# alexlee-gk/video_prediction

Hardware: AMD Instinct MI355X
Metric: train frames/sec (whole node), BAIR 64x64 seq30 SAVP (higher is better)
Workload: dtype bf16

## Files before the change

### include/savp_hip.h

```cpp
#ifndef SAVP_HIP_H
#define SAVP_HIP_H

#include <stdint.h>

#ifdef __cplusplus
extern "C" {
#endif

#define SAVP_OK 0
#define SAVP_EINVAL (-1)
#define SAVP_ELAUNCH (-2)

const char* savp_version(void);

int savp_set_option(const char* name, int32_t value);
int savp_get_option(const char* name, int32_t* value);

int savp_allreduce_bucket(void* comm, void* stream, void* buf, int64_t count);

int savp_prof_event_create(void** ev);
int savp_prof_event_destroy(void* ev);
int savp_prof_arm(void* start, void* stop);
int savp_prof_armed(void);
int savp_prof_elapsed_us(void* start, void* stop, float* us);

enum { SAVP_CONV_FPROP = 0, SAVP_CONV_DGRAD = 1, SAVP_CONV_WGRAD = 2 };
enum { SAVP_PREC_F32 = 0, SAVP_PREC_BF16 = 1 };
enum { SAVP_ACT_NONE = 0, SAVP_ACT_LRELU = 1, SAVP_ACT_SIGMOID = 2, SAVP_ACT_DLRELU_FROM_OUT = 3 };

typedef struct SavpConvArgs {
    int32_t mode;
    int32_t N, D, H, W, Cx;
    int32_t Do, Ho, Wo, Cy;
    int32_t kd, kh, kw;
    int32_t sd, sh, sw;
    int32_t pd, ph, pw;
    int32_t beta;
    int32_t act;
    float alpha;
    int32_t splitk;
    int32_t tile;
    int32_t precision;
    void* x; int64_t x_sn, x_sd, x_sh, x_sw;
    void* y; int64_t y_sn, y_sd, y_sh, y_sw;
    void* w;
    const float* bias;
    const float* aux;
    const void* w_bf16;
    int32_t src_bf16;
    int32_t out_bf16;
    double* stats;
    void* ws; int64_t ws_bytes;
    int32_t dst_gap_at, dst_gap;
    const float* nb_x; int64_t nb_x_sn, nb_x_sp;
    const float *nb_mean, *nb_rstd;
    const float *nb_gamma, *nb_beta;
    double* nb_ws;
    int32_t nb_c0, nb_nc, nb_act; float nb_alpha;
    const void* w_frag;
    const void* w_frag_il;
} SavpConvArgs;

int savp_conv(void* stream, const SavpConvArgs* args);

int savp_tiled_z_weff(void* stream, const float* w, int32_t kh, int32_t kw, int32_t ph, int32_t pw, int32_t Cin, int32_t Cout,
                      int32_t z0, int32_t nz, float* weff);
int savp_tiled_z_grad(void* stream, const void* dy, int32_t dy_bf16, int64_t nimg, int32_t H, int32_t W, int32_t C,
                      const float* weff, int32_t nz, float* dz, int32_t beta, void* ws, int64_t ws_bytes);
int64_t savp_tiled_z_workspace_bytes(int64_t nimg, int32_t C);
int savp_conv_stats_ok(const SavpConvArgs* args);
int64_t savp_conv_workspace_bytes(const SavpConvArgs* args);
int savp_conv_special(const SavpConvArgs* args);


typedef struct SavpView { void* p; int64_t sn; int64_t sp; } SavpView;

typedef struct SavpInormArgs {
    int32_t N, HW, C;
    int32_t act; float alpha; float eps;
    SavpView x;
    const float* gamma; const float* beta;
    int32_t nout; SavpView out[4];
    float* mean; float* rstd;
    int32_t ndy; SavpView dy[4];
    SavpView dx; int32_t dx_beta;
    double* dgamma; double* dbeta;
    void* ws;
    int32_t ws_clean;
    int32_t out_c0[4], out_nc[4];
    int32_t dy_c0[4], dy_nc[4];
    int32_t out_bf16;
    int32_t stats_ready;
    const float* stats_shift;
    int32_t dx_bf16;
} SavpInormArgs;
int savp_instnorm_act_fwd(void* stream, const SavpInormArgs* a);
int savp_instnorm_act_bwd(void* stream, const SavpInormArgs* a);

typedef struct SavpGnormArgs {
    SavpInormArgs norm;
    int32_t G;
    double* ws_group;
    double* dsum;
} SavpGnormArgs;
int savp_groupnorm_act_fwd(void* stream, const SavpGnormArgs* a);
int savp_groupnorm_act_bwd(void* stream, const SavpGnormArgs* a);

typedef struct SavpLnLstmArgs {
    int32_t N, HW, F; float forget_bias;
    const float* gn;
    SavpView c_prev;
    float* c_pre;
    const float* cn;
    int32_t nh; SavpView h[4]; int32_t h_bf16;
    int32_t ndh; SavpView dh[4];
    const float* dc_new;
    float* dcn;
    float* dgn;
    const float* dc_pre;
    float* dc_prev;
} SavpLnLstmArgs;
int savp_lnlstm_fwd(void* stream, const SavpLnLstmArgs* a, int32_t stage);
int savp_lnlstm_bwd(void* stream, const SavpLnLstmArgs* a, int32_t stage);

typedef struct SavpLstmArgs {
    int32_t N, HW, F;
    float eps, forget_bias;
    const void* gates;
    SavpView c_prev;
    const float *gamma1, *beta1, *gamma2, *beta2;
    float* c_new;
    int32_t nh; SavpView h[4];
    float *mean1, *rstd1, *mean2, *rstd2;
    int32_t ndh; SavpView dh[4];
    const float* dc_new;
    float* dgates;
    float* dc_prev;
    double *dgamma1, *dbeta1, *dgamma2, *dbeta2;
    float* ws; int64_t ws_floats;
    float* ws_stats;
    int32_t ws_stats_clean;
    int32_t gates_bf16;
    int32_t stats1_ready;
// ... 200 lines not shown
    float* du;
    SavpView dh;
    SavpView drh;
    double *dgamma, *dbeta;
} SavpGruArgs;
int savp_convgru_gates_fwd(void* stream, const SavpGruArgs* a);
int savp_convgru_out_fwd(void* stream, const SavpGruArgs* a);
int savp_convgru_out_bwd(void* stream, const SavpGruArgs* a);
int savp_convgru_gates_bwd(void* stream, const SavpGruArgs* a);

int savp_u8_frames_to_f32(void* stream, const uint8_t* in, float* out, int32_t B, int32_t T, int64_t frame);
int savp_u8_frames_resize_f32(void* stream, const uint8_t* in, float* out, int32_t B, int32_t T, int32_t Hs, int32_t Ws, int32_t C,
                              int32_t crop, int32_t S);

typedef struct SavpJpegArgs {
    int32_t N;
    int32_t width, height, components;
    int32_t h[3], v[3], blocks_w[3], blocks_h[3], block_offset[3], total_blocks;
    int32_t out_h, out_w;
    const int16_t* coef;
    const uint16_t* qtab;
    const int32_t* window;
    uint8_t* out;
    void* ws; int64_t ws_bytes;
} SavpJpegArgs;
int savp_jpeg_decode_u8(void* stream, const SavpJpegArgs* a);
int64_t savp_jpeg_workspace_bytes(const SavpJpegArgs* a);

int savp_frame_mse_psnr(void* stream, const float* a, int64_t a_st, int64_t a_sb, const float* b, int64_t b_st, int64_t b_sb,
                        int32_t T, int32_t B, int32_t inner, float* mse, float* psnr);
int savp_frame_ssim(void* stream, const float* a, int64_t a_st, int64_t a_sb, const float* b, int64_t b_st, int64_t b_sb,
                    int32_t T, int32_t B, int32_t H, int32_t W, int32_t C, float* out);
int savp_eval_accumulate(void* stream, const float* metric, float* vmin, float* vsum, float* vmax, int32_t* cond_min,
                         int32_t* cond_max, int32_t T, int32_t B);
int savp_select_batch(void* stream, const int32_t* cond, const float* x, int64_t x_st, int64_t x_sb, float* out, int64_t o_st,
                      int64_t o_sb, int32_t T, int32_t B, int32_t inner, int32_t mode);

#define SAVP_EVAL_PSNR 0
#define SAVP_EVAL_MSE 1
#define SAVP_EVAL_SSIM 2
#define SAVP_EVAL_NMETRICS 3
typedef struct {
    float *vmin, *vsum, *vmax;
    float *gmin, *gsum, *gmax;
} SavpEvalFoldState;
int64_t savp_eval_fold_ws_floats(int32_t F, int32_t S, int32_t B, int32_t C);
int savp_eval_fold_samples(void* stream, const float* target, int64_t t_st, int64_t t_sb, const float* pred, int64_t p_st, int64_t p_sb,
                           int32_t F, int32_t T1, int32_t S, int32_t B, int32_t H, int32_t W, int32_t C, const int32_t* n_valid,
                           const SavpEvalFoldState* states, float* ws, int64_t ws_floats);

int savp_eval_fold_metric(void* stream, const float* metric, const float* pred, int64_t p_st, int64_t p_sb, int32_t F, int32_t T1,
                          int32_t S, int32_t B, int32_t inner, const int32_t* n_valid, const SavpEvalFoldState* state, int32_t* sel);

#define SAVP_LPIPS_TAPS 5
#define SAVP_LPIPS_STEM_CO 64
#define SAVP_LPIPS_STEM_KROW 36
int savp_lpips_stem(void* stream, const float* x, int64_t x_s0, int64_t x_s1, int32_t N, int32_t N1, int32_t H, int32_t W, int32_t C,
                    const float* wp, const float* bias, float* y);
int savp_lpips_maxpool3s2(void* stream, const float* x, int32_t N, int32_t H, int32_t W, int32_t C, float* y);
typedef struct {
    int32_t F, N;
    int32_t hw[SAVP_LPIPS_TAPS], c[SAVP_LPIPS_TAPS];
    const float* a[SAVP_LPIPS_TAPS];
    const float* b[SAVP_LPIPS_TAPS];
    const float* lin[SAVP_LPIPS_TAPS];
    int32_t a_n1, b_n1, b_mod, out_n1;
    float sign;
    float* out;
    const int32_t* ctl;
    int32_t B, s0, nd;
} SavpLpipsHeadArgs;
int savp_lpips_head(void* stream, const SavpLpipsHeadArgs* a);
int savp_lpips_diversity_add(void* stream, const float* dv, int32_t F, int32_t S, int32_t B, const int32_t* ctl, int32_t nd, float* div);

int savp_fold_f64(void* stream, const int32_t* idx, int64_t n, double* src, float* dst);

int savp_state_pred_fwd(void* stream, int32_t T, int32_t N, int32_t na, int32_t ns, const float* actions, const float* states_in,
                        const int32_t* gt, const float* W, const float* b, float* sa, float* gen);
int savp_state_pred_bwd(void* stream, int32_t T, int32_t N, int32_t na, int32_t ns, const int32_t* gt, const float* W, const float* sa,
                        float* dgen, double* dW, double* db);

int64_t savp_gate_weights_bytes(int32_t taps, int32_t Cx, int32_t Cy);
int savp_pack_gate_weights(void* stream, const float* src, int32_t taps, int32_t Cx, int32_t Cy, void* out, int32_t interleave);

int savp_debug_poison_lds(void* stream, uint32_t pattern, void* sink);
int savp_debug_fill_u32(void* stream, void* p, int64_t words, uint32_t pattern);
int savp_debug_probe_lds(void* stream, uint32_t pattern, void* out2);

#ifdef __cplusplus
}
#endif
#endif
```

### video_prediction_amd/csrc/common.hip

```cpp
#include <hip/hip_runtime.h>
#include <dlfcn.h>
#include <string.h>
#include "savp_hip.h"
#include "opts.h"
#include "conv_common.h"

extern "C" const char* savp_version(void) { return "savp_hip 0.1 gfx950"; }

thread_local hipEvent_t g_savp_prof_start = nullptr;
thread_local hipEvent_t g_savp_prof_stop = nullptr;

extern "C" int savp_prof_event_create(void** ev) {
    if (!ev) return SAVP_EINVAL;
    hipEvent_t e;
    if (hipEventCreate(&e) != hipSuccess) return SAVP_ELAUNCH;
    *ev = (void*)e;
    return SAVP_OK;
}
extern "C" int savp_prof_event_destroy(void* ev) { return (ev && hipEventDestroy((hipEvent_t)ev) == hipSuccess) ? SAVP_OK : SAVP_EINVAL; }
extern "C" int savp_prof_arm(void* start, void* stop) {
    if ((start == nullptr) != (stop == nullptr)) return SAVP_EINVAL;
    g_savp_prof_start = (hipEvent_t)start; g_savp_prof_stop = (hipEvent_t)stop;
    return SAVP_OK;
}
extern "C" int savp_prof_armed(void) { return g_savp_prof_start != nullptr; }
extern "C" int savp_prof_elapsed_us(void* start, void* stop, float* us) {
    if (!start || !stop || !us) return SAVP_EINVAL;
    float ms = 0.f;
    if (hipEventElapsedTime(&ms, (hipEvent_t)start, (hipEvent_t)stop) != hipSuccess) return SAVP_ELAUNCH;
    *us = ms * 1e3f;
    return SAVP_OK;
}

static struct { const char* name; int value; } g_opts[OPT_COUNT] = {
    {"conv_ring", 0}, {"s2dgrad", 1}, {"thin", 1}, {"wgp_cfg", 0}, {"wgp_split", 0}, {"inorm_min_hw", 64}, {"colsum_2stage", 1},
    {"dense_legacy", 0}, {"cdna_legacy", 0}, {"lstm_fused", 1}, {"ring_dma", 1}, {"lstm_q", 0}, {"ring_wwarm", 1}, {"wgp_dma", 1}, {"ring_early", 1}, {"gate_kernel", 1}, {"gate_alt", 0}, {"gate_cell", 1}, {"gate_wwarm", 1}, {"splitk_reduced", 0},
};
int savp_opt(int id) { return g_opts[id].value; }
void savp_opt_count(int id) { ++g_opts[id].value; }
extern "C" int savp_set_option(const char* name, int value) {
    if (!name) return SAVP_EINVAL;
    for (int i = 0; i < OPT_COUNT; ++i)
        if (!strcmp(g_opts[i].name, name)) { g_opts[i].value = value; return SAVP_OK; }
    return SAVP_EINVAL;
}
extern "C" int savp_get_option(const char* name, int* value) {
    if (!name || !value) return SAVP_EINVAL;
    for (int i = 0; i < OPT_COUNT; ++i)
        if (!strcmp(g_opts[i].name, name)) { *value = g_opts[i].value; return SAVP_OK; }
    return SAVP_EINVAL;
}

typedef int (*rccl_allreduce_fn)(const void*, void*, size_t, int, int, void*, hipStream_t);
extern "C" int savp_allreduce_bucket(void* comm, void* stream, void* buf, int64_t count) {
    if (!comm || !buf || count < 0) return SAVP_EINVAL;
    if (count == 0) return SAVP_OK;
    static rccl_allreduce_fn fn = nullptr;
    if (!fn) {
        void* h = dlopen("librccl.so", RTLD_NOW | RTLD_GLOBAL);
        if (!h) h = dlopen("librccl.so.1", RTLD_NOW | RTLD_GLOBAL);
        if (!h) h = dlopen("/opt/rocm/lib/librccl.so", RTLD_NOW | RTLD_GLOBAL);
        if (!h) return SAVP_ELAUNCH;
        fn = (rccl_allreduce_fn)dlsym(h, "ncclAllReduce");
        if (!fn) return SAVP_ELAUNCH;
    }
    return fn(buf, buf, (size_t)count, 7, 0, comm, (hipStream_t)stream) == 0 ? SAVP_OK : SAVP_ELAUNCH;
}

int splitk_fit(const SavpConvArgs* a, int want, long long block_elems) {
    if (want <= 1) return 1;
    if (!a->ws || a->ws_bytes <= 0 || block_elems <= 0 || (((uintptr_t)a->ws) & 15)) { savp_opt_count(OPT_SPLITK_REDUCED); return 1; }
    const long long fit = a->ws_bytes / (block_elems * (long long)sizeof(float));
    if (fit < want) savp_opt_count(OPT_SPLITK_REDUCED);
    if (fit < 2) return 1;
    return want < fit ? want : (int)fit;
}

__global__ __launch_bounds__(256) void splitk_fold_kernel(float* __restrict__ out, const float* __restrict__ part, int splitk, long long n4, long long n,
                                                          int beta, int Cd, int gap_at, int gap) {
    const long long stride = (long long)gridDim.x * 256;
    for (long long i = (long long)blockIdx.x * 256 + threadIdx.x; i < n4; i += stride) {
        float4 s = beta ? reinterpret_cast<const float4*>(out)[i] : make_float4(0.f, 0.f, 0.f, 0.f);
        for (int k = 0; k < splitk; ++k) {
            const float4 v = reinterpret_cast<const float4*>(part + (long long)k * n)[i];
            s.x += v.x; s.y += v.y; s.z += v.z; s.w += v.w;
        }
        if (gap) {
            const int c = (int)((i * 4) % Cd);
            float* e = &s.x;
#pragma unroll
            for (int j = 0; j < 4; ++j)
                if (c + j >= gap_at && c + j < gap_at + gap) e[j] = beta ? reinterpret_cast<const float*>(out)[i * 4 + j] : 0.f;
        }
        reinterpret_cast<float4*>(out)[i] = s;
    }
}

__global__ __launch_bounds__(256) void splitk_fold_scalar_kernel(float* __restrict__ out, const float* __restrict__ part, int splitk, long long n, int beta,
                                                                 int Cd, int gap_at, int gap) {
    const long long stride = (long long)gridDim.x * 256;
    for (long long i = (long long)blockIdx.x * 256 + threadIdx.x; i < n; i += stride) {
        const int c = (int)(i % Cd);
        if (gap && c >= gap_at && c < gap_at + gap) { if (!beta) out[i] = 0.f; continue; }
        float s = beta ? out[i] : 0.f;
        for (int k = 0; k < splitk; ++k) s += part[(long long)k * n + i];
        out[i] = s;
    }
}

void splitk_fold(float* out, const float* part, int splitk, long long n, int beta, int Cd, int gap_at, int gap, hipStream_t st) {
    const bool vec = (n % 4 == 0) && (Cd % 4 == 0) && ((((uintptr_t)out) & 15) == 0) && ((((uintptr_t)part) & 15) == 0);
    const long long work = vec ? n / 4 : n;
    long long blocks = (work + 255) / 256;
    if (blocks > 2048) blocks = 2048;
    if (blocks < 1) blocks = 1;
    if (vec) hipLaunchKernelGGL(splitk_fold_kernel, dim3((unsigned)blocks), dim3(256), 0, st, out, part, splitk, n / 4, n, beta, Cd, gap_at, gap);
    else hipLaunchKernelGGL(splitk_fold_scalar_kernel, dim3((unsigned)blocks), dim3(256), 0, st, out, part, splitk, n, beta, Cd, gap_at, gap);
}

// ... 36 lines not shown
```

### video_prediction_amd/csrc/conv_common.h

```cpp
#pragma once
#include <hip/hip_runtime.h>
#include <stdint.h>
#include "savp_hip.h"
#include "opts.h"

typedef float f32x16 __attribute__((ext_vector_type(16)));
typedef __bf16 bf16x8 __attribute__((ext_vector_type(8)));
typedef __bf16 bf16x4 __attribute__((ext_vector_type(4)));

#define BK 32
#define BKP 36
#define NTHREADS 256

struct DimGeom {
    int Mdim;
    int base, mstep;
    int jstep;
    int nt;
    int t0, tstep;
    int ob, os;
    int srcN;
};

__host__ __device__ __forceinline__ DimGeom make_geom(bool dgrad, int f, int In, int Out, int k, int s, int p) {
// ... 44 lines not shown
    int pre;
    const float* nb_x; long long nb_x_sn, nb_x_sp; const float *nb_mean, *nb_rstd, *nb_gamma, *nb_beta; double* nb_ws;
    int nb_c0, nb_nc, nb_act; float nb_alpha;
    int gap_at, gap;
    int wwarm;
    int early;
    DimGeom gD, gH, gW;
    int s1_tih_sh;
    int s1_ngs, s1_itper;
    unsigned long long s1_magTm, s1_magTHW, s1_magTW;
    unsigned long long s1_magKw, s1_magSpp, s1_magTail;
};

__device__ __forceinline__ unsigned fastdiv(unsigned p, unsigned long long magic) {
    return (unsigned)(((unsigned long long)p * magic) >> 40);
}

__device__ __forceinline__ float4 ldg4(const float* p) { return *reinterpret_cast<const float4*>(p); }

__device__ __forceinline__ int xcd_logical(int b, int n) {
    const int q = n >> 3, r = n & 7, xcd = b & 7;
    return (xcd < r ? xcd * (q + 1) : r * (q + 1) + (xcd - r) * q) + (b >> 3);
}


static inline unsigned long long magic40(int d) {
    if (d <= 0) d = 1;
    return ((1ULL << 40) + (unsigned long long)d - 1ULL) / (unsigned long long)d;
}

static inline void patch_launch_constants(ConvP& p, const SavpConvArgs* a, int phases, int tih, int nch, int spp, int tW, int splitk) {
    const bool dg = a->mode == SAVP_CONV_DGRAD;
    int sh_ = 0;
    while ((1 << sh_) < tih) ++sh_;
    p.s1_tih_sh = sh_;
    const int ngs = (nch + spp - 1) / spp;
    p.s1_ngs = ngs;
    p.pre = 0;
    if (phases != 1 || (dg && (a->sh != 1 || a->sw != 1))) return;
    p.gD = make_geom(dg, 0, a->D, a->Do, a->kd, 1, a->pd);
    p.gH = make_geom(dg, 0, a->H, a->Ho, a->kh, a->sh, a->ph);
    p.gW = make_geom(dg, 0, a->W, a->Wo, a->kw, a->sw, a->pw);
    const long long it_all = (long long)p.gD.nt * p.gH.nt * p.gW.nt * nch;
    p.s1_itper = (int)((it_all + splitk - 1) / splitk);
    const int thw = p.s1_th * tW;
    p.s1_magTm = magic40(p.tm); p.s1_magTHW = magic40(thw); p.s1_magTW = magic40(tW);
    p.s1_magKw = magic40(p.gW.nt); p.s1_magSpp = magic40(spp); p.s1_magTail = magic40(nch - (ngs - 1) * spp);
    if ((long long)p.tm * p.tn < (1 << 24) && p.tm < 65536 && thw < 65536 && it_all < (1 << 24) && p.gW.nt >= 1 && p.gH.nt >= 1) p.pre = 1;
}

bool conv_thin_try(const SavpConvArgs* a, hipStream_t st, int* rc);
bool conv_thin_applies(const SavpConvArgs* a);
long long conv_thin_workspace_bytes(const SavpConvArgs* a);

bool conv_s2dgrad_try(const SavpConvArgs* a, hipStream_t st, int* rc);
bool conv_s2dgrad_applies(const SavpConvArgs* a);

extern thread_local hipEvent_t g_savp_prof_start, g_savp_prof_stop;

int splitk_fit(const SavpConvArgs* a, int want, long long block_elems);
void splitk_fold(float* out, const float* part, int splitk, long long n, int beta, int Cd, int gap_at, int gap, hipStream_t st);

static inline bool aligned16(const void* p) { return (((uintptr_t)p) & 15) == 0; }

#ifdef SAVP_CONV_ABLATE
#include <stdlib.h>
static __constant__ int g_ablate;
#define ABL(bit) (g_ablate & (bit))
static inline void ablate_init() {
    static bool done = false;
    if (!done) { const char* e = getenv("SAVP_ABLATE"); int v = e ? atoi(e) : 0; hipMemcpyToSymbol(HIP_SYMBOL(g_ablate), &v, sizeof(int)); done = true; }
}
#else
#define ABL(bit) false
static inline void ablate_init() {}
#endif

bool conv_patch_try(ConvP& p, const SavpConvArgs* a, int wm, int wn, bool forced, hipStream_t st, int* rc);
bool conv_wgrad_patch_try(ConvP& p, const SavpConvArgs* a, hipStream_t st, int* rc, long long* plan_bytes = nullptr);
void wgrad_fold(float* out, const float* part, int nsplit, long long n, hipStream_t st, long long slice = 0);
bool conv_ring_try(ConvP& p, const SavpConvArgs* a, int wm, int wn, hipStream_t st, int* rc, bool dry = false);
bool conv_gate_applies(const SavpConvArgs* a);
bool conv_gate_try(const SavpConvArgs* a, hipStream_t st, int* rc);
struct SavpConvLstmCellArgs;
bool conv_gate_cell_try(const SavpConvLstmCellArgs* c, hipStream_t st, int* rc);
```

### video_prediction_amd/csrc/conv_gate.hip

```cpp
#include "conv_common.h"
#include "opts.h"
#include <hip/hip_ext.h>
#include <type_traits>

extern thread_local hipEvent_t g_savp_prof_start;
extern thread_local hipEvent_t g_savp_prof_stop;

struct GateP {
    const unsigned short* x;
    const uint4* wfrag;
    unsigned short* y;
    double* stats;
    const void* zero16;
    int N, Cy, mtiles, ntiles;
    int wwarm;
    int F; float eps, forget_bias;
    const float* c_prev; long long cp_sn, cp_sp;
    const float *g1, *b1, *g2, *b2;
    float* c_new;
    int nh; void* h[4]; long long h_sn[4], h_sp[4]; int h16;
    float *mean1, *rstd1, *mean2, *rstd2;
};

__device__ __attribute__((aligned(16))) unsigned g_gate_zero[4] = {0u, 0u, 0u, 0u};

#ifdef SAVP_GATE_STAMPS
__device__ unsigned long long g_gate_t[4][8];
__constant__ int g_gate_blk = 0;
#define GT(i) do { if ((int)blockIdx.x == g_gate_blk && (threadIdx.x & 63) == 0) g_gate_t[threadIdx.x >> 6][i] = __builtin_readcyclecounter(); } while (0)
extern "C" int savp_debug_gate_times(unsigned long long* out) { return hipMemcpyFromSymbol(out, HIP_SYMBOL(g_gate_t), sizeof(g_gate_t)) == hipSuccess ? 0 : -1; }
extern "C" int savp_debug_gate_block(int b) { return hipMemcpyToSymbol(HIP_SYMBOL(g_gate_blk), &b, sizeof(int)) == hipSuccess ? 0 : -1; }
#else
#define GT(i) do {} while (0)
#endif

__device__ __forceinline__ void gate_touch4(const void* gsrc, unsigned lds_dst) {
    unsigned keep;
    asm volatile("s_mov_b32 %0, m0\n\ts_mov_b32 m0, %2\n\ts_nop 0\n\tglobal_load_lds_dword %1, off\n\ts_mov_b32 m0, %0"
                 : "=&s"(keep) : "v"(gsrc), "s"(lds_dst) : "memory");
}

__device__ __forceinline__ void gate_dma16(const void* gsrc, unsigned lds_dst) {
    unsigned keep;
    asm volatile("s_mov_b32 %0, m0\n\ts_mov_b32 m0, %2\n\ts_nop 0\n\tglobal_load_lds_dwordx4 %1, off\n\ts_mov_b32 m0, %0"
                 : "=&s"(keep) : "v"(gsrc), "s"(lds_dst) : "memory");
}

template <int S, int CIN, int TM, int TN, int NWN>
struct GateCfg {
    static constexpr int KH = 5, KW = 5, PAD = 2, TAPS = KH * KW;
    static constexpr int KSPLIT = 4 / NWN;
    static constexpr int PIX = 32 * TM;
    static constexpr int C8 = CIN / 8;
    static constexpr int C8P = (C8 & 1) ? C8 : C8 + 1;
    static constexpr int PXB = C8P * 16;
    static constexpr int TC = S >= 16 ? 16 : 8;
    static constexpr int TR = (S * S >= PIX) ? PIX / TC : S;
    static constexpr int NI = PIX / (TR * TC);
    static constexpr int PR = TR + 2 * PAD, PC = TC + 2 * PAD;
    static constexpr int RPAD = (256 - (4 * PXB) % 256) % 256;
    static constexpr int RP = PC * PXB + RPAD;
    static constexpr int IMGB = PR * RP;
    static constexpr int PATCHB = NI * IMGB;
    static constexpr int NCH = TAPS * C8;
    static constexpr int KS = (NCH + 1) / 2;
    static constexpr int KPAD = 8;
    static constexpr int ETABB = ((2 * (KS + KPAD) * 4) + 15) & ~15;
    static constexpr int NCW = 32 * TN;
    static constexpr int NC = NCW * NWN;
    static constexpr int TILEB = 32 * 32 * 4;
    static constexpr int XB = (KSPLIT > 1 ? TM / 2 : 0) * TN * TILEB;
    static constexpr int TP = NC / 2 + 4;
    static constexpr int STGB = PIX * TP * 4;
    static constexpr int STATB = KSPLIT * NC * 2 * 4;
    static constexpr int EPIB = (4 * XB > STGB ? 4 * XB : STGB) + STATB;
    static constexpr int WARMB = 256;
    static constexpr int LDSB = (PATCHB + ETABB + WARMB) > EPIB ? (PATCHB + ETABB + WARMB) : EPIB;
    static constexpr int TPI = NI == 1 ? (S / TR) * (S / TC) : 1;
    static constexpr int PPR = PC * C8P;
    static constexpr int NJ = (PPR + 63) / 64;
    static constexpr int aoff(int i) { return ((i * 32) / (TR * TC)) * IMGB + (((i * 32) % (TR * TC)) / TC) * RP; }
    static_assert(CIN % 8 == 0 && S % TC == 0 && S % TR == 0 && (TM == 4 || TM == 8) && (TN == 1 || TN == 2) && (NWN == 1 || NWN == 2) && TR * TC * NI == PIX && 32 % TC == 0, "shape");
    static_assert(LDSB <= 160 * 1024, "LDS");
};

template <int TM, int TN, int I>
__device__ __forceinline__ void gate_sched() {
    constexpr int M = TM * TN, ND = TM + 1, NV = TN;
    if constexpr (I < M) {
        constexpr int d = (ND * (I + 1)) / M - (ND * I) / M;
        constexpr int v = (NV * (I + 1)) / M - (NV * I) / M;
        if constexpr (d > 0) __builtin_amdgcn_sched_group_barrier(0x100, d, 0);
        if constexpr (v > 0) __builtin_amdgcn_sched_group_barrier(0x020, v, 0);
        __builtin_amdgcn_sched_group_barrier(0x008, 1, 0);
        gate_sched<TM, TN, I + 1>();
    }
}

template <int S, int CIN, int TM, int TN, int NWN, bool CELL = false>
__global__ __launch_bounds__(256, (2 * GateCfg<S, CIN, TM, TN, NWN>::LDSB <= 160 * 1024 ? 2 : 1)) void conv_gate_kernel(GateP p) {
    GT(0);
    using G = GateCfg<S, CIN, TM, TN, NWN>;
    constexpr int KS = G::KS, NC = G::NC;
    extern __shared__ __attribute__((aligned(16))) unsigned char gsm[];
    unsigned char* patch = gsm;
    unsigned* etab = reinterpret_cast<unsigned*>(gsm + G::PATCHB);
    const int tid = threadIdx.x, lane = tid & 63;
    const int wave = __builtin_amdgcn_readfirstlane(tid >> 6);
    const int nw = wave % NWN, kq = wave / NWN;
    constexpr int KSPLIT = G::KSPLIT;
    const int l31 = lane & 31, khalf = lane >> 5;

    const int logical = xcd_logical((int)blockIdx.x, p.mtiles * p.ntiles);
    const int nt = logical / p.mtiles, mt = logical - nt * p.mtiles;
    const int n0 = nt * NC;
    int img0, ty0, tx0;
    if constexpr (G::NI == 1) {
        img0 = mt / G::TPI;
        const int tr = mt % G::TPI;
        ty0 = (tr / (S / G::TC)) * G::TR; tx0 = (tr % (S / G::TC)) * G::TC;
    } else {
        img0 = mt * G::NI; ty0 = 0; tx0 = 0;
    }

    if (p.wwarm) {
        const int nwg = p.mtiles * p.ntiles, qx = nwg >> 3, rx = nwg & 7, xcd = (int)blockIdx.x & 7;
        const int first = xcd < rx ? xcd * (qx + 1) : rx * (qx + 1) + (xcd - rx) * qx;
        const int cnt = qx + (xcd < rx ? 1 : 0);
        const int l_lo = max(first, nt * p.mtiles), l_hi = min(first + cnt, (nt + 1) * p.mtiles);
        const int share = max(l_hi - l_lo, 1), mine = min(max(logical - l_lo, 0), share - 1);
        constexpr int BLK = TN * NWN * KS * 1024;
        const int chunk = ((BLK + share - 1) / share + 8191) & ~8191;
        const unsigned char* wb = reinterpret_cast<const unsigned char*>(p.wfrag) + (size_t)(n0 / 32) * KS * 1024;
        const unsigned warm_lds = (unsigned)(uintptr_t)(gsm + G::PATCHB + G::ETABB);
        for (int off = wave * 8192; off < chunk && mine * chunk + off < BLK; off += 4 * 8192) {
            const int a = min(mine * chunk + off + lane * 128, BLK - 4);
            gate_touch4(wb + a, warm_lds);
        }
    }
    {
        const unsigned patch_lds = (unsigned)(uintptr_t)patch;
        const unsigned char* xb = reinterpret_cast<const unsigned char*>(p.x);
        const unsigned long long zero16 = (unsigned long long)(uintptr_t)p.zero16;
        int rel[G::NJ];
#pragma unroll
        for (int j = 0; j < G::NJ; ++j) {
            const int piece = j * 64 + lane;
            const int px = piece / G::C8P, ch = piece - px * G::C8P;
            const int ix = tx0 + px - G::PAD;
            const bool ok = piece < G::PPR && ch < G::C8 && (unsigned)ix < (unsigned)S;
            rel[j] = ok ? (ix * CIN + ch * 8) * 2 : -1;
        }
        for (int row = wave; row < G::NI * G::PR; row += 4) {
            const int im = row / G::PR, py = row - im * G::PR;
            const int n = img0 + im, iy = ty0 + py - G::PAD;
            const bool row_ok = (unsigned)iy < (unsigned)S && n < p.N;
            const unsigned char* rb = xb + ((long long)n * S + iy) * (long long)(S * CIN * 2);
            const unsigned lds_row = patch_lds + (unsigned)(im * G::IMGB + py * G::RP);
            if (!row_ok) {
#pragma unroll
                for (int j = 0; j < G::NJ; ++j)
                    if (j * 64 + lane < G::PPR) *reinterpret_cast<uint4*>(patch + im * G::IMGB + py * G::RP + (j * 64 + lane) * 16) = make_uint4(0u, 0u, 0u, 0u);
                continue;
            }
#pragma unroll
            for (int j = 0; j < G::NJ; ++j) {
                if (j * 64 + lane < G::PPR) {
                    const unsigned long long g = (row_ok && rel[j] >= 0) ? (unsigned long long)(uintptr_t)(rb + rel[j]) : zero16;
                    gate_dma16(reinterpret_cast<const void*>((uintptr_t)g), lds_row + (unsigned)(j * 1024));
                }
            }
        }
    }
    GT(1);
    for (int c = tid; c < 2 * (KS + G::KPAD); c += 256) {
        const int cc = c < G::NCH ? c : 0;
        const int tap = cc / G::C8, ch = cc - tap * G::C8;
        etab[c] = (unsigned)((tap / G::KW) * G::RP + (tap % G::KW) * G::PXB + ch * 16);
    }

    constexpr int KSW = (KS + KSPLIT - 1) / KSPLIT;
    const int ks0 = kq * KSW, ks1 = min(KS, ks0 + KSW);
    const uint4* __restrict__ bsrc[TN];
#pragma unroll
    for (int j = 0; j < TN; ++j) bsrc[j] = p.wfrag + ((long long)(n0 / 32 + nw * TN + j) * KS) * 64 + lane;
    constexpr int PF = (TM * TN >= 8) ? 4 : 8;
#ifndef SAVP_GATE_ABL
#define SAVP_GATE_ABL 0
#endif
    uint4 bq[PF][TN];
#pragma unroll
    for (int u = 0; u < PF; ++u)
#pragma unroll
        for (int j = 0; j < TN; ++j) bq[u][j] = bsrc[j][(long long)(ks0 + u) * 64];

    const unsigned a0 = (unsigned)((l31 / G::TC) * G::RP + (l31 % G::TC) * G::PXB);
    f32x16 acc[TM][TN];
#pragma unroll
    for (int i = 0; i < TM; ++i)
#pragma unroll
        for (int j = 0; j < TN; ++j)
#pragma unroll
            for (int r = 0; r < 16; ++r) acc[i][j][r] = 0.f;

    GT(2);
    asm volatile("s_waitcnt vmcnt(0)" ::: "memory");
    __syncthreads();
    GT(3);

    bf16x8 af[2][TM];
    auto load_a = [&](bf16x8 (&dst)[TM], unsigned off) {
        const unsigned char* a = patch + a0 + off;
#pragma unroll
        for (int i = 0; i < TM; ++i) dst[i] = *reinterpret_cast<const bf16x8*>(a + G::aoff(i));
    };
    const unsigned* etl = etab + khalf;
    load_a(af[0], etl[2 * ks0]);
    unsigned off_next = etl[2 * (ks0 + 1)];
    auto kstep = [&](int k, auto uc, auto steadyc) {
        constexpr int u = decltype(uc)::value;
        constexpr bool STEADY = decltype(steadyc)::value;
        if (!(SAVP_GATE_ABL & 2)) {
            load_a(af[(u + 1) & 1], off_next);
            off_next = etl[2 * (k + 2)];
        }
        bf16x8 bf[TN];
#pragma unroll
        for (int j = 0; j < TN; ++j) bf[j] = __builtin_bit_cast(bf16x8, bq[u % PF][j]);
#pragma unroll
        for (int i = 0; i < TM; ++i)
#pragma unroll
            for (int j = 0; j < TN; ++j) {
                if (!(SAVP_GATE_ABL & 4)) acc[i][j] = __builtin_amdgcn_mfma_f32_32x32x16_bf16(af[u & 1][i], bf[j], acc[i][j], 0, 0, 0);
                else asm volatile("" :: "v"(af[u & 1][i]), "v"(bf[j]));
            }
        if (!(SAVP_GATE_ABL & 1)) {
#pragma unroll
            for (int j = 0; j < TN; ++j) bq[u % PF][j] = bsrc[j][(long long)(k + PF) * 64];
        }
        if constexpr (STEADY) gate_sched<TM, TN, 0>();
    };
    using U0 = std::integral_constant<int, 0>; using U1 = std::integral_constant<int, 1>;
    using U2 = std::integral_constant<int, 2>; using U3 = std::integral_constant<int, 3>;
    using U4 = std::integral_constant<int, 4>; using U5 = std::integral_constant<int, 5>;
    using U6 = std::integral_constant<int, 6>; using U7 = std::integral_constant<int, 7>;
    static_assert(PF == 4 || PF == 8, "the loop is unrolled PF k-steps: the B ring's slots are compile-time registers");
    int k = ks0;
    auto body = [&](auto... us) { (kstep(k + decltype(us)::value, us, std::true_type{}), ...); };
    auto tail = [&](auto... us) { ((k < ks1 ? (kstep(k, us, std::false_type{}), ++k, 0) : 0), ...); };
    if constexpr (PF == 4) {
        for (; k + 4 <= ks1; k += 4) body(U0{}, U1{}, U2{}, U3{});
        tail(U0{}, U1{}, U2{});
    } else {
        for (; k + 8 <= ks1; k += 8) body(U0{}, U1{}, U2{}, U3{}, U4{}, U5{}, U6{}, U7{});
        tail(U0{}, U1{}, U2{}, U3{}, U4{}, U5{}, U6{});
    }
    GT(4);

    __syncthreads();
    constexpr int TMH = TM / 2, TMQ = TM / 4;
    float4* xbuf = reinterpret_cast<float4*>(gsm);
    auto xput = [&](int wslot, auto ilo_c, auto ni_c) {
        constexpr int ILO = decltype(ilo_c)::value, NI_ = decltype(ni_c)::value;
        float4* dst = xbuf + (size_t)wslot * (G::XB / 16) + lane;
#pragma unroll
        for (int i = ILO; i < ILO + NI_; ++i)
#pragma unroll
            for (int j = 0; j < TN; ++j)
#pragma unroll
                for (int g = 0; g < 4; ++g) {
                    dst[(((i - ILO) * TN + j) * 4 + g) * 64] = make_float4(acc[i][j][4 * g], acc[i][j][4 * g + 1], acc[i][j][4 * g + 2], acc[i][j][4 * g + 3]);
                    if (g == 3) __builtin_amdgcn_sched_barrier(0);
                }
    };
    auto xadd = [&](int wslot, auto ilo_c, auto ni_c) {
        constexpr int ILO = decltype(ilo_c)::value, NI_ = decltype(ni_c)::value;
        const float4* src = xbuf + (size_t)wslot * (G::XB / 16) + lane;
#pragma unroll
        for (int i = ILO; i < ILO + NI_; ++i)
#pragma unroll
            for (int j = 0; j < TN; ++j)
#pragma unroll
                for (int g = 0; g < 4; ++g) {
                    const float4 v = src[(((i - ILO) * TN + j) * 4 + g) * 64];
                    acc[i][j][4 * g] += v.x; acc[i][j][4 * g + 1] += v.y; acc[i][j][4 * g + 2] += v.z; acc[i][j][4 * g + 3] += v.w;
                    if (g == 3) __builtin_amdgcn_sched_barrier(0);
// ... 116 lines not shown
                }
                float gk[4];
#pragma unroll
                for (int k = 0; k < 4; ++k) {
                    float b[4];
#pragma unroll
                    for (int t = 0; t < 4; ++t) {
                        const int ai = __builtin_bit_cast(int, a4[t]);
                        const int bi = k == 0 ? __builtin_amdgcn_mov_dpp(ai, 0x00, 0xF, 0xF, true) : k == 1 ? __builtin_amdgcn_mov_dpp(ai, 0x55, 0xF, 0xF, true)
                                     : k == 2 ? __builtin_amdgcn_mov_dpp(ai, 0xAA, 0xF, 0xF, true) : __builtin_amdgcn_mov_dpp(ai, 0xFF, 0xF, 0xF, true);
                        b[t] = __builtin_bit_cast(float, bi);
                    }
                    gk[k] = g == 0 ? b[0] : (g == 1 ? b[1] : (g == 2 ? b[2] : b[3]));
                }
                const float c = cp[i * 4 + m] * gk[2] + gk[0] * gk[1];
                cpre[i * 4 + m] = c; so[i * 4 + m] = gk[3];
                s2 += c; q2 += c * c;
            }
        s2 += __shfl_xor(s2, 1); q2 += __shfl_xor(q2, 1);
        s2 += __shfl_xor(s2, 2); q2 += __shfl_xor(q2, 2);
        s2 += __shfl_xor(s2, 32); q2 += __shfl_xor(q2, 32);
        if (khalf == 0 && g == 0) { stat2[(kq * 8 + ch) * 2] = s2; stat2[(kq * 8 + ch) * 2 + 1] = q2; }
        asm volatile("s_waitcnt lgkmcnt(0)" ::: "memory");
        __builtin_amdgcn_s_barrier();
        float mu2, rs2;
        {
            float t0 = 0.f, t1 = 0.f;
#pragma unroll
            for (int o = 0; o < WPI; ++o) {
                const int ord = im * WPI + o, w = ((ord & 1) << 1) | (ord >> 1);
                t0 += stat2[(w * 8 + ch) * 2]; t1 += stat2[(w * 8 + ch) * 2 + 1];
            }
            const double m = (double)t0 * (double)inv;
            mu2 = (float)m;
            rs2 = rsqrtf(fmaxf((float)((double)t1 * (double)inv - m * m), 0.f) + p.eps);
        }
        if (live && kq == first_of_image && khalf == 0 && g == 0) { p.mean2[(long long)n * F + cch] = mu2; p.rstd2[(long long)n * F + cch] = rs2; }
        GT(6);
        if (live && !(SAVP_CELL_ABL & 2)) {
            const float sc2 = rs2 * ga2, sh2 = be2 - mu2 * rs2 * ga2;
            float cn[NE], hv[NE];
#pragma unroll
            for (int e = 0; e < NE; ++e) {
                cn[e] = cpre[e] * sc2 + sh2;
                const float ee = __expf(-2.f * fabsf(cn[e]));
                hv[e] = copysignf((1.f - ee) * __builtin_amdgcn_rcpf(1.f + ee), cn[e]) * so[e];
            }
            float* __restrict__ cb = p.c_new + (long long)n * HWI * F + cch;
#pragma unroll
            for (int i = 0; i < TMFc; ++i)
#pragma unroll
                for (int m = 0; m < 4; ++m) cb[(erow(i, m) % HWI) * F] = cn[i * 4 + m];
#pragma unroll
            for (int k = 0; k < 4; ++k) {
                if (k >= p.nh) break;
                const int hsp = (int)p.h_sp[k];
                if ((p.h16 >> k) & 1) {
                    unsigned short* __restrict__ hb = reinterpret_cast<unsigned short*>(p.h[k]) + (long long)n * p.h_sn[k] + cch;
#pragma unroll
                    for (int i = 0; i < TMFc; ++i)
#pragma unroll
                        for (int m = 0; m < 4; ++m) hb[(erow(i, m) % HWI) * hsp] = __builtin_bit_cast(unsigned short, (__bf16)hv[i * 4 + m]);
                } else {
                    float* __restrict__ hb = reinterpret_cast<float*>(p.h[k]) + (long long)n * p.h_sn[k] + cch;
#pragma unroll
                    for (int i = 0; i < TMFc; ++i)
#pragma unroll
                        for (int m = 0; m < 4; ++m) hb[(erow(i, m) % HWI) * hsp] = hv[i * 4 + m];
                }
            }
        }
        for (int idx = tid; idx < G::PIX * 4; idx += 256) {
            const int pix = idx >> 2, gg = idx & 3;
            const int imp = pix / HWI, px = pix - imp * HWI;
            const int np = img0 + imp;
            if (np >= p.N) continue;
            const uint4 w = *reinterpret_cast<const uint4*>(T16 + pix * 32 + gg * 8);
            *reinterpret_cast<uint4*>(p.y + ((long long)np * HWI + px) * (long long)p.Cy + gg * F + nt * 8) = w;
        }
        GT(7);
        return;
    }

    float* stat = reinterpret_cast<float*>(gsm + (4 * G::XB > G::STGB ? 4 * G::XB : G::STGB));
    unsigned* T = reinterpret_cast<unsigned*>(gsm);
    constexpr int TMF = TM / KSPLIT;
    auto finish = [&](auto fin_c) {
        constexpr int FIN = decltype(fin_c)::value;
        const bool oddl = lane & 1;
#pragma unroll
        for (int i = FIN; i < FIN + TMF; ++i)
#pragma unroll
            for (int j = 0; j < TN; ++j) {
                const int cp = (nw * G::NCW + 32 * j + (l31 & ~1)) >> 1;
#pragma unroll
                for (int m = 0; m < 8; ++m) {
                    const float e = acc[i][j][2 * m], o = acc[i][j][2 * m + 1];
                    const float en = __builtin_bit_cast(float, __builtin_amdgcn_mov_dpp(__builtin_bit_cast(int, e), 0xB1, 0xF, 0xF, true));
                    const float on = __builtin_bit_cast(float, __builtin_amdgcn_mov_dpp(__builtin_bit_cast(int, o), 0xB1, 0xF, 0xF, true));
                    const int r = 2 * m + (oddl ? 1 : 0);
                    const int row = i * 32 + (r & 3) + 8 * (r >> 2) + 4 * khalf;
                    typedef __bf16 bf16x2 __attribute__((ext_vector_type(2)));
                    T[row * G::TP + cp] = oddl ? __builtin_bit_cast(unsigned, bf16x2{(__bf16)on, (__bf16)o}) : __builtin_bit_cast(unsigned, bf16x2{(__bf16)e, (__bf16)en});
                }
            }
        if (p.stats) {
#pragma unroll
            for (int j = 0; j < TN; ++j) {
                float sm = 0.f, q = 0.f;
#pragma unroll
                for (int i = FIN; i < FIN + TMF; ++i)
#pragma unroll
                    for (int r = 0; r < 16; ++r) { const float v = acc[i][j][r]; sm += v; q += v * v; }
                sm += __shfl_xor(sm, 32); q += __shfl_xor(q, 32);
                if (khalf == 0) { stat[(kq * NC + nw * G::NCW + 32 * j + l31) * 2] = sm; stat[(kq * NC + nw * G::NCW + 32 * j + l31) * 2 + 1] = q; }
            }
        }
    };
    if constexpr (KSPLIT == 4) {
        if (!odd && !hi) finish(IC0{});
        else if (!odd && hi) finish(ICQ{});
        else if (odd && !hi) finish(ICH{});
        else finish(ICHQ{});
    } else {
        if (!odd) finish(IC0{}); else finish(ICH{});
    }
    __syncthreads();
    GT(6);
    {
        constexpr int CH = NC / 8;
        for (int idx = tid; idx < G::PIX * CH; idx += 256) {
            const int pix = idx / CH, c8 = idx - pix * CH;
            const int im = pix / (G::TR * G::TC), rr = pix - im * (G::TR * G::TC);
            const int n = img0 + im;
            if (n >= p.N) continue;
            const int oy = ty0 + rr / G::TC, ox = tx0 + rr % G::TC;
            const uint4 v = *reinterpret_cast<const uint4*>(T + pix * G::TP + c8 * 4);
            unsigned short* dst = p.y + (((long long)n * S + oy) * S + ox) * (long long)p.Cy + n0 + c8 * 8;
            *reinterpret_cast<uint4*>(dst) = v;
        }
    }
    if (p.stats) {
        constexpr int WPI = KSPLIT / G::NI;
        for (int i = tid; i < G::NI * NC * 2; i += 256) {
            const int im = i / (NC * 2), rem = i - im * (NC * 2);
            const int n = img0 + im;
            if (n >= p.N) continue;
            float t = 0.f;
#pragma unroll
            for (int o = 0; o < WPI; ++o) {
                const int ord = im * WPI + o;
                const int q_ = KSPLIT == 4 ? (((ord & 1) << 1) | (ord >> 1)) : ord;
                t += stat[q_ * NC * 2 + rem];
            }
            unsafeAtomicAdd(p.stats + ((long long)n * p.Cy + n0 + (rem >> 1)) * 2 + (rem & 1), (double)t);
        }
    }
    GT(7);
}

#define GATE_PACK_PAD_KSTEPS 8
__global__ __launch_bounds__(256) void pack_gate_weights_kernel(const float* __restrict__ src, int taps, int Cx, int Cy, uint4* __restrict__ out, int il_F) {
    const int C8 = Cx >> 3, nch = taps * C8, KS = (nch + 1) >> 1;
    const long long total = (long long)(Cy >> 5) * KS * 64;
    for (long long t = total + (long long)blockIdx.x * 256 + threadIdx.x; t < total + GATE_PACK_PAD_KSTEPS * 64; t += (long long)gridDim.x * 256)
        out[t] = make_uint4(0u, 0u, 0u, 0u);
    for (long long t = (long long)blockIdx.x * 256 + threadIdx.x; t < total; t += (long long)gridDim.x * 256) {
        const int lane = (int)(t & 63);
        const long long r = t >> 6;
        const int ks = (int)(r % KS), cb = (int)(r / KS);
        const int c = 2 * ks + (lane >> 5);
        typedef __bf16 bf16x2 __attribute__((ext_vector_type(2)));
        unsigned w[4] = {0u, 0u, 0u, 0u};
        if (c < nch) {
            const int tap = c / C8, ch = c - tap * C8;
            const int l = lane & 31, col = il_F ? (l & 3) * il_F + cb * 8 + (l >> 2) : cb * 32 + l;
            const float* s = src + ((long long)tap * Cx + ch * 8) * Cy + col;
#pragma unroll
            for (int j = 0; j < 4; ++j) w[j] = __builtin_bit_cast(unsigned, bf16x2{(__bf16)s[(long long)(2 * j) * Cy], (__bf16)s[(long long)(2 * j + 1) * Cy]});
        }
        out[t] = make_uint4(w[0], w[1], w[2], w[3]);
    }
}

extern "C" int64_t savp_gate_weights_bytes(int32_t taps, int32_t Cx, int32_t Cy) {
    if (taps < 1 || Cx < 8 || (Cx & 7) || Cy < 32 || (Cy & 31)) return 0;
    const long long KS = ((long long)taps * (Cx >> 3) + 1) >> 1;
    return ((long long)(Cy >> 5) * KS + GATE_PACK_PAD_KSTEPS) * 64 * 16;
}

extern "C" int savp_pack_gate_weights(void* stream, const float* src, int32_t taps, int32_t Cx, int32_t Cy, void* out, int32_t interleave) {
    if (!src || !out || !savp_gate_weights_bytes(taps, Cx, Cy) || (((uintptr_t)out) & 15)) return SAVP_EINVAL;
    if (interleave && (Cy % 4 != 0 || (Cy / 4) % 8 != 0)) return SAVP_EINVAL;
    const long long total = savp_gate_weights_bytes(taps, Cx, Cy) / 16 - GATE_PACK_PAD_KSTEPS * 64;
    unsigned nb = (unsigned)((total + 255) / 256);
    if (nb > 4096) nb = 4096;
    hipLaunchKernelGGL(pack_gate_weights_kernel, dim3(nb), dim3(256), 0, (hipStream_t)stream, src, taps, Cx, Cy, (uint4*)out, interleave ? Cy / 4 : 0);
    return hipGetLastError() == hipSuccess ? SAVP_OK : SAVP_ELAUNCH;
}

template <int S, int CIN, int TM, int TN, int NWN, bool CELL = false>
static hipError_t launch_gate(const GateP& p, hipStream_t st) {
    using G = GateCfg<S, CIN, TM, TN, NWN>;
    static bool attr = false;
    if (!attr) {
        hipFuncSetAttribute((const void*)conv_gate_kernel<S, CIN, TM, TN, NWN, CELL>, hipFuncAttributeMaxDynamicSharedMemorySize, G::LDSB);
        attr = true;
    }
    const dim3 grid((unsigned)(p.mtiles * p.ntiles));
    if (g_savp_prof_start) {
        hipExtLaunchKernelGGL((conv_gate_kernel<S, CIN, TM, TN, NWN, CELL>), grid, dim3(256), G::LDSB, st, g_savp_prof_start, g_savp_prof_stop, 0, p);
        g_savp_prof_start = g_savp_prof_stop = nullptr;
    } else {
        hipLaunchKernelGGL((conv_gate_kernel<S, CIN, TM, TN, NWN, CELL>), grid, dim3(256), G::LDSB, st, p);
    }
    return hipGetLastError();
}

#define GATE_SHAPES(X)                                                                                                    \
    X(32, 72, 8, 1, 2, 0) X(16, 136, 4, 1, 1, 0) X(8, 264, 4, 1, 1, 0)        \
    X(32, 96, 8, 1, 2, 0) X(16, 160, 4, 1, 1, 0)                            \
    X(32, 64, 8, 1, 2, 0) X(16, 128, 4, 1, 1, 0) X(8, 256, 4, 1, 1, 0)      \
    X(32, 136, 8, 1, 2, 0) X(32, 264, 4, 1, 2, 0) X(16, 264, 4, 1, 2, 0)    \
    X(32, 72, 4, 1, 2, 1) X(16, 136, 4, 1, 2, 2) X(32, 96, 4, 1, 2, 1) X(16, 160, 4, 1, 2, 2) X(32, 72, 4, 1, 1, 4) X(32, 72, 4, 2, 1, 8)

static bool gate_shape_ok(const SavpConvArgs* a) {
#define X(S_, C_, TM_, TN_, NWN_, ALT_) if (a->H == S_ && a->Cx == C_) return true;
    GATE_SHAPES(X)
#undef X
    return false;
}

bool conv_gate_applies(const SavpConvArgs* a) {
    if (!savp_opt(OPT_GATE_KERNEL)) return false;
    if (!(a->mode == SAVP_CONV_FPROP && a->precision == SAVP_PREC_BF16 && a->src_bf16 && a->out_bf16 && a->w_frag && !a->bias && !a->aux &&
          a->act == SAVP_ACT_NONE && !a->beta && !a->dst_gap && !a->nb_ws && a->splitk <= 1))
        return false;
    if (!(a->D == 1 && a->Do == 1 && a->kd == 1 && a->kh == 5 && a->kw == 5 && a->sd == 1 && a->sh == 1 && a->sw == 1 && a->pd == 0 && a->ph == 2 &&
          a->pw == 2 && a->H == a->W && a->Ho == a->H && a->Wo == a->W))
        return false;
    if (!(a->x_sw == a->Cx && a->x_sh == (long long)a->W * a->Cx && a->x_sn == (long long)a->H * a->W * a->Cx && a->y_sw == a->Cy &&
          a->y_sh == (long long)a->W * a->Cy && a->y_sn == (long long)a->H * a->W * a->Cy && aligned16(a->x) && aligned16(a->y) && aligned16(a->w_frag)))
        return false;
    if ((a->Cy & 127) || a->N < 1 || (a->stats && (((uintptr_t)a->stats) & 7))) return false;
    return gate_shape_ok(a);
}

bool conv_gate_try(const SavpConvArgs* a, hipStream_t st, int* rc) {
    if (!conv_gate_applies(a)) return false;
    static const void* zero_of[64] = {nullptr};
    int dev_ord = 0;
    if (hipGetDevice(&dev_ord) != hipSuccess || dev_ord < 0 || dev_ord >= 64) dev_ord = 0;
    if (!zero_of[dev_ord] && hipGetSymbolAddress((void**)&zero_of[dev_ord], HIP_SYMBOL(g_gate_zero)) != hipSuccess) { *rc = SAVP_ELAUNCH; return true; }
    GateP p;
    p.x = (const unsigned short*)a->x; p.wfrag = (const uint4*)a->w_frag; p.y = (unsigned short*)a->y; p.stats = (double*)a->stats;
    p.zero16 = zero_of[dev_ord]; p.N = a->N; p.Cy = a->Cy; p.wwarm = savp_opt(OPT_GATE_WWARM);
    hipError_t err = hipErrorInvalidValue;
    const int alt = savp_opt(OPT_GATE_ALT);
    bool done = false;
#define X(S_, C_, TM_, TN_, NWN_, ALT_)                                                                  \
    if (!done && a->H == S_ && a->Cx == C_ && (want ? (ALT_ & want) != 0 : ALT_ == 0)) {                 \
        using G = GateCfg<S_, C_, TM_, TN_, NWN_>;                                                       \
        p.mtiles = G::NI == 1 ? a->N * G::TPI : (a->N + G::NI - 1) / G::NI; p.ntiles = a->Cy / G::NC;    \
        err = launch_gate<S_, C_, TM_, TN_, NWN_>(p, st);                                                \
        done = true;                                                                                     \
    }
    { const int want = alt; GATE_SHAPES(X) }
    { const int want = 0; GATE_SHAPES(X) }
#undef X
    *rc = err == hipSuccess ? SAVP_OK : SAVP_ELAUNCH;
    return true;
}

#define GATE_CELL_SHAPES(X) X(16, 136, 8) X(8, 264, 4) X(16, 160, 8) X(16, 128, 8) X(8, 256, 4)

bool conv_gate_cell_try(const SavpConvLstmCellArgs* c, hipStream_t st, int* rc) {
    const SavpConvArgs* a = &c->conv;
    const SavpLstmArgs* g = &c->gates;
    if (!savp_opt(OPT_GATE_KERNEL) || !savp_opt(OPT_GATE_CELL) || !a->w_frag_il) return false;
    SavpConvArgs b = *a;
    b.w_frag = a->w_frag_il;
    if (!b.stats) b.stats = (double*)(uintptr_t)16;
    if (!conv_gate_applies(&b)) return false;
    bool shape = false;
#define X(S_, C_, TM_) if (a->H == S_ && a->Cx == C_) shape = true;
    GATE_CELL_SHAPES(X)
#undef X
    if (!shape) return false;
    if (g->no_norm || !g->gates_bf16 || g->F * 4 != a->Cy || g->N != a->N || g->HW != a->H * a->W || g->nh < 0 || g->nh > 4 || !g->gamma1 || !g->beta1 ||
        !g->gamma2 || !g->beta2 || !g->c_new || !g->mean1 || !g->rstd1 || !g->mean2 || !g->rstd2 || (g->F & 7))
        return false;
    if (g->c_prev.sp * (long long)g->HW >= (1ll << 31)) return false;
    for (int i = 0; i < g->nh; ++i)
        if (g->h[i].sp * (long long)g->HW >= (1ll << 31)) return false;
    static const void* zero_of[64] = {nullptr};
    int dev_ord = 0;
    if (hipGetDevice(&dev_ord) != hipSuccess || dev_ord < 0 || dev_ord >= 64) dev_ord = 0;
    if (!zero_of[dev_ord] && hipGetSymbolAddress((void**)&zero_of[dev_ord], HIP_SYMBOL(g_gate_zero)) != hipSuccess) { *rc = SAVP_ELAUNCH; return true; }
    GateP p;
    p.x = (const unsigned short*)a->x; p.wfrag = (const uint4*)a->w_frag_il; p.y = (unsigned short*)a->y; p.stats = nullptr;
    p.zero16 = zero_of[dev_ord]; p.N = a->N; p.Cy = a->Cy; p.wwarm = savp_opt(OPT_GATE_WWARM);
    p.F = g->F; p.eps = g->eps; p.forget_bias = g->forget_bias;
    p.c_prev = (const float*)g->c_prev.p; p.cp_sn = g->c_prev.sn; p.cp_sp = g->c_prev.sp;
    p.g1 = g->gamma1; p.b1 = g->beta1; p.g2 = g->gamma2; p.b2 = g->beta2;
    p.c_new = g->c_new; p.nh = g->nh; p.h16 = g->h_bf16;
    for (int i = 0; i < 4; ++i) { p.h[i] = i < g->nh ? g->h[i].p : nullptr; p.h_sn[i] = i < g->nh ? g->h[i].sn : 0; p.h_sp[i] = i < g->nh ? g->h[i].sp : 0; }
    p.mean1 = g->mean1; p.rstd1 = g->rstd1; p.mean2 = g->mean2; p.rstd2 = g->rstd2;
    hipError_t err = hipErrorInvalidValue;
#define X(S_, C_, TM_)                                                                                   \
    if (a->H == S_ && a->Cx == C_) {                                                                     \
        using G = GateCfg<S_, C_, TM_, 1, 1>;                                                            \
        p.mtiles = (a->N + G::NI - 1) / G::NI; p.ntiles = a->Cy / 32;                                    \
        err = launch_gate<S_, C_, TM_, 1, 1, true>(p, st);                                               \
    }
    GATE_CELL_SHAPES(X)
#undef X
    *rc = err == hipSuccess ? SAVP_OK : SAVP_ELAUNCH;
    return true;
}
```

### video_prediction_amd/csrc/conv_igemm.hip

```cpp
#include <hip/hip_runtime.h>
#include <stdint.h>
#include "savp_hip.h"
#include "zero_fill.h"

#include "conv_common.h"
#include <stdlib.h>

template <int WM, int WN, bool VEC, bool BF16, bool WB16>
__global__ __launch_bounds__(NTHREADS) void conv_fd_kernel(ConvP p) {
    constexpr int BM = 64 * WM, BN = 64 * WN;
    constexpr int BKT = BF16 ? 64 : 32;
    constexpr int KV = BKT / 4;
    constexpr int RP = NTHREADS / KV;
    constexpr int RA = BM / RP, RB = BN / RP;
    constexpr int ROWB = BF16 ? (BKT + 8) * 2 : BKP * 4;
    extern __shared__ __attribute__((aligned(16))) float smem[];
    char* As = reinterpret_cast<char*>(smem);
    char* Bs = As + 2 * BM * ROWB;

    const bool dgrad = (p.mode == SAVP_CONV_DGRAD);
    const int split = blockIdx.z % p.splitk;
    int fz = blockIdx.z / p.splitk;
    int fw = dgrad ? fz % p.sw : 0; fz = dgrad ? fz / p.sw : 0;
    int fh = dgrad ? fz % p.sh : 0; fz = dgrad ? fz / p.sh : 0;
// ... 669 lines not shown
        double rounds = wgs <= 256.0 ? 1.0 : wgs / 256.0;
        double eff = (bm * bn == 128 * 128) ? 1.0 : (bm * bn == 64 * 64 ? 1.3 : 1.12);
        double cost = rounds * (double)(bm * bn) * eff;
        if (cost < best) { best = cost; wm = opts[i][0]; wn = opts[i][1]; }
    }
}

static bool ring_default() {
    return savp_opt(OPT_CONV_RING) != 0;
}

struct WgPlan { int wm, wn, splitk; long long M, ktiles, part_sz; bool va, vb, wbf16; };
static bool wgrad_generic_plan(const SavpConvArgs* a, bool bf16, int wm, int wn, WgPlan& g) {
    const bool xs4 = (a->x_sn % 4 == 0) && (a->x_sd % 4 == 0) && (a->x_sh % 4 == 0) && (a->x_sw % 4 == 0) && aligned16(a->x);
    const bool ys4 = (a->y_sn % 4 == 0) && (a->y_sd % 4 == 0) && (a->y_sh % 4 == 0) && (a->y_sw % 4 == 0) && aligned16(a->y);
    g.M = (long long)a->kd * a->kh * a->kw * a->Cx;
    const long long Ktot = (long long)a->N * a->Do * a->Ho * a->Wo;
    if (Ktot <= 0 || (double)Ktot * (double)((long long)a->Do * a->Ho * a->Wo) >= 1099511627776.0) return false;
    g.va = (a->Cx % 4 == 0) && xs4;
    g.vb = (a->Cy % 4 == 0) && ys4;
    if (!wm) {
        wm = (g.M > 64) ? 2 : 1;
        wn = (a->Cy > 64) ? 2 : 1;
    }
    g.wm = wm; g.wn = wn;
    const int BM = 64 * wm, BN = 64 * wn;
    const long long tiles = ((g.M + BM - 1) / BM) * ((a->Cy + BN - 1) / BN);
    g.wbf16 = bf16 && g.va && g.vb;
    const int bkt = g.wbf16 ? 64 : BK;
    g.ktiles = (Ktot + bkt - 1) / bkt;
    long long splitk = a->splitk;
    if (splitk <= 0) {
        long long want = (512 + tiles - 1) / tiles;
        long long maxs = g.ktiles / 8 > 0 ? g.ktiles / 8 : 1;
        splitk = want < maxs ? want : maxs;
    }
    if (splitk > g.ktiles) splitk = g.ktiles;
    if (splitk < 1) splitk = 1;
    const long long per = (g.ktiles + splitk - 1) / splitk;
    g.splitk = (int)((g.ktiles + per - 1) / per);
    g.part_sz = g.M * a->Cy;
    return true;
}

extern "C" int64_t savp_conv_workspace_bytes(const SavpConvArgs* a) {
    if (!a) return 0;
    if (a->mode == SAVP_CONV_FPROP || a->mode == SAVP_CONV_DGRAD) {
        if (a->act != SAVP_ACT_NONE || a->out_bf16 || a->stats || a->splitk == 1) return 0;
        const bool dg = a->mode == SAVP_CONV_DGRAD;
        const long long dD = dg ? a->D : a->Do, dH = dg ? a->H : a->Ho, dW_ = dg ? a->W : a->Wo;
        const long long Cd = (dg ? a->Cx : a->Cy) + (a->dst_gap > 0 ? a->dst_gap : 0);
        const long long block = (long long)a->N * dD * dH * dW_ * Cd;
        long long S = a->splitk;
        if (S <= 0) {
            const long long tiles = ((block / Cd + 255) / 256) * ((Cd + 127) / 128);
            if (tiles > 192) return 0;
            S = 512 / tiles;
            if (S > 16) S = 16;
        }
        return S > 1 ? S * block * (long long)sizeof(float) : 0;
    }
    if (a->mode != SAVP_CONV_WGRAD) return 0;
    const int algo = (a->tile >> 8) & 3;
    long long need = 0;
    const long long thin = algo == 0 ? conv_thin_workspace_bytes(a) : 0;
    if (thin) need = thin;
    else {
        int wm = 0, wn = 0;
        if (a->tile & 0xff) { wm = (a->tile >> 4) & 15; wn = a->tile & 15; if (wm < 1 || wm > 2 || wn < 1 || wn > 2) return 0; }
        ConvP p;
        p.bf16 = (a->precision == SAVP_PREC_BF16) ? 1 : 0;
        int rc = SAVP_OK;
        long long patch_bytes = 0;
        WgPlan g;
        if (algo != 1 && conv_wgrad_patch_try(p, a, nullptr, &rc, &patch_bytes)) need = patch_bytes;
        else if (algo != 2 && wgrad_generic_plan(a, p.bf16 != 0, wm, wn, g) && g.splitk > 1) need = (long long)g.splitk * g.part_sz * (long long)sizeof(float);
        const long long bias = a->bias ? (long long)SAVP_COLSUM_WS_FLOATS * 4 : 0;
        if (bias > need) need = bias;
    }
    return need;
}

extern "C" int savp_conv_special(const SavpConvArgs* a) {
    if (a && conv_gate_applies(a)) return 1;
    if (!a || ((a->tile >> 8) & 3) != 0) return 0;
    return (conv_thin_applies(a) || conv_s2dgrad_applies(a) || conv_gate_applies(a)) ? 1 : 0;
}

extern "C" int savp_conv_stats_ok(const SavpConvArgs* a) {
    if (!a || (a->mode != SAVP_CONV_FPROP && a->mode != SAVP_CONV_DGRAD) || a->precision != SAVP_PREC_BF16) return 0;
    if (((a->tile >> 8) & 3) == 0 && (conv_thin_applies(a) || conv_s2dgrad_applies(a))) return 0;
    const bool dg = a->mode == SAVP_CONV_DGRAD;
    const int Cred = dg ? a->Cy : a->Cx;
    if (!(a->w_bf16 && (Cred % 8 == 0) && aligned16(a->w_bf16))) return 0;
    ConvP p;
    p.bf16 = 1; p.w16 = (const unsigned short*)a->w_bf16; p.src16 = a->src_bf16 ? 1 : 0; p.splitk = 1; p.tm = p.tn = 1;
    p.gap_at = a->dst_gap ? a->dst_gap_at : 0x7fffffff; p.gap = a->dst_gap;
    p.nb_ws = (double*)a->nb_ws; p.nb_c0 = a->nb_c0; p.nb_nc = a->nb_nc; p.part = nullptr; p.part_sz = 0;
    if (a->dst_gap && !a->nb_ws) return 0;
    if (a->nb_ws && (a->nb_act < 0 || a->nb_act > 2)) return 0;
    SavpConvArgs b = *a;
    if (!b.stats && !b.nb_ws) b.stats = (double*)(uintptr_t)16;
    int wm = 0, wn = 0;
    if (b.tile & 0xff) { wm = (b.tile >> 4) & 15; wn = b.tile & 15; if (wm < 1 || wm > 2 || wn < 1 || wn > 2) return 0; }
    int rc = SAVP_OK;
    return conv_ring_try(p, &b, wm, wn, nullptr, &rc, true) ? 1 : 0;
}

extern "C" int savp_conv(void* stream, const SavpConvArgs* a) {
    if (!a || !a->x || !a->y || !a->w) return SAVP_EINVAL;
    if (a->sd < 1 || a->sh < 1 || a->sw < 1 || a->kd < 1 || a->kh < 1 || a->kw < 1) return SAVP_EINVAL;
    hipStream_t st = (hipStream_t)stream;
    ConvP p;
    p.mode = a->mode;
    p.N = a->N; p.D = a->D; p.H = a->H; p.W = a->W; p.Cx = a->Cx;
    p.Do = a->Do; p.Ho = a->Ho; p.Wo = a->Wo; p.Cy = a->Cy;
    p.kd = a->kd; p.kh = a->kh; p.kw = a->kw; p.sd = a->sd; p.sh = a->sh; p.sw = a->sw;
    p.pd = a->pd; p.ph = a->ph; p.pw = a->pw;
    p.beta = a->beta; p.act = a->act; p.alpha = a->alpha;
    p.x = (const float*)a->x; p.x_sn = a->x_sn; p.x_sd = a->x_sd; p.x_sh = a->x_sh; p.x_sw = a->x_sw;
    p.y = (const float*)a->y; p.y_sn = a->y_sn; p.y_sd = a->y_sd; p.y_sh = a->y_sh; p.y_sw = a->y_sw;
    p.w = (const float*)a->w;
    p.w16 = nullptr;
    p.bias = a->bias; p.aux = a->aux;
    p.splitk = 1; p.tm = p.tn = 1; p.part = nullptr; p.part_sz = 0;
    p.src16 = a->src_bf16 ? 1 : 0; p.cell = 0; p.stats = nullptr;
    p.bf16 = (a->precision == SAVP_PREC_BF16) ? 1 : 0;
    const bool gapped = a->dst_gap != 0;
    if (gapped && (a->dst_gap < 0 || a->dst_gap_at < 0 || a->mode == SAVP_CONV_WGRAD)) return SAVP_EINVAL;
    p.gap_at = gapped ? a->dst_gap_at : 0x7fffffff; p.gap = gapped ? a->dst_gap : 0;
    p.nb_ws = (double*)a->nb_ws;
    if (a->nb_ws) {
        if (a->mode == SAVP_CONV_WGRAD || !a->nb_x || !a->nb_mean || !a->nb_rstd || !a->nb_gamma || !a->nb_beta || a->nb_c0 < 0 || a->nb_nc < 1 ||
            a->nb_act < 0 || a->nb_act > 2)
            return SAVP_EINVAL;
        p.nb_x = a->nb_x; p.nb_x_sn = a->nb_x_sn; p.nb_x_sp = a->nb_x_sp; p.nb_mean = a->nb_mean; p.nb_rstd = a->nb_rstd;
        p.nb_gamma = a->nb_gamma; p.nb_beta = a->nb_beta; p.nb_c0 = a->nb_c0; p.nb_nc = a->nb_nc; p.nb_act = a->nb_act; p.nb_alpha = a->nb_alpha;
    }
    p.magW = magic40(a->Wo); p.magHW = magic40(a->Ho * a->Wo); p.magDHW = magic40(a->Do * a->Ho * a->Wo);
    int wm = 0, wn = 0;
    const int algo = (a->tile >> 8) & 3;
    if (a->tile & 0xff) { wm = (a->tile >> 4) & 15; wn = a->tile & 15; if (wm < 1 || wm > 2 || wn < 1 || wn > 2) return SAVP_EINVAL; }
    hipError_t err;
    ablate_init();
    const bool xs4 = (a->x_sn % 4 == 0) && (a->x_sd % 4 == 0) && (a->x_sh % 4 == 0) && (a->x_sw % 4 == 0) && aligned16(a->x);
    const bool ys4 = (a->y_sn % 4 == 0) && (a->y_sd % 4 == 0) && (a->y_sh % 4 == 0) && (a->y_sw % 4 == 0) && aligned16(a->y);
    if (algo == 0 && !gapped && !a->nb_ws) {
        int rc = SAVP_OK;
        if (conv_thin_try(a, st, &rc)) return rc;
    }
    if (algo == 0 && !gapped && !a->nb_ws && a->mode == SAVP_CONV_DGRAD) {
        int rc = SAVP_OK;
        if (conv_s2dgrad_try(a, st, &rc)) return rc;
    }
    if (a->mode == SAVP_CONV_FPROP) {
        int rc = SAVP_OK;
        if (conv_gate_try(a, st, &rc)) return rc;
    }
    if (a->mode == SAVP_CONV_FPROP || a->mode == SAVP_CONV_DGRAD) {
        const bool dg = a->mode == SAVP_CONV_DGRAD;
        p.out = (float*)(dg ? a->x : a->y);
        const int Cred = dg ? a->Cy : a->Cx;
        const int Nout = dg ? a->Cx : a->Cy;
        const bool vec = (Cred % 4 == 0) && (dg ? ys4 : xs4) && aligned16(a->w);
        if (a->w_bf16 && (Cred % 8 == 0) && aligned16(a->w_bf16)) p.w16 = (const unsigned short*)a->w_bf16;
        long long Mmax;
        int phases = 1;
        if (dg) {
            phases = a->sd * a->sh * a->sw;
            Mmax = (long long)a->N * ((a->D + a->sd - 1) / a->sd) * ((a->H + a->sh - 1) / a->sh) * ((a->W + a->sw - 1) / a->sw);
        } else {
            Mmax = (long long)a->N * a->Do * a->Ho * a->Wo;
        }
        if (Mmax <= 0 || Nout <= 0) return SAVP_EINVAL;
        const bool needs_ring = a->out_bf16 || a->src_bf16 || a->stats || gapped || a->nb_ws;
        if (algo == 3 || needs_ring || (algo == 0 && ring_default())) {
            int rc = SAVP_OK;
            if (conv_ring_try(p, a, wm, wn, st, &rc)) return rc;
            if (algo == 3 || needs_ring) return SAVP_EINVAL;
        }
        if (algo != 1) {
            int rc = SAVP_OK;
            if (conv_patch_try(p, a, wm, wn, algo == 2, st, &rc)) return rc;
            if (algo == 2) return SAVP_EINVAL;
        }
        if (!wm) pick_tile(Mmax * phases, Nout, wm, wn);
        const int BM = 64 * wm, BN = 64 * wn;
        int splitk = a->splitk;
        const long long tiles = ((Mmax + BM - 1) / BM) * ((Nout + BN - 1) / BN) * phases;
        const long long taps_max = (long long)a->kd * a->kh * a->kw / (dg ? phases : 1);
        const long long nkt = (taps_max * Cred + (p.bf16 ? 63 : 31)) / (p.bf16 ? 64 : 32);
        const bool can_split = (a->act == SAVP_ACT_NONE);
        if (!can_split) splitk = 1;
        else if (splitk <= 0) {
            splitk = 1;
            if (tiles <= 192 && nkt >= 16) {
                long long s1 = 512 / tiles, s2 = nkt / 8;
                splitk = (int)(s1 < s2 ? s1 : s2);
                if (splitk < 1) splitk = 1;
                if (splitk > 16) splitk = 16;
            }
        }
        if (splitk > 1) {
            const long long dD = dg ? a->D : a->Do, dH = dg ? a->H : a->Ho, dW_ = dg ? a->W : a->Wo;
            const long long s_n = dg ? a->x_sn : a->y_sn, s_d = dg ? a->x_sd : a->y_sd, s_h = dg ? a->x_sh : a->y_sh,
                            s_w = dg ? a->x_sw : a->y_sw;
            const bool dense = (s_w == Nout) && (s_h == dW_ * Nout) && (dD == 1 || s_d == dH * dW_ * Nout) &&
                               (s_n == dD * dH * dW_ * Nout);
            if (!dense) splitk = 1;
            else {
                p.part_sz = (long long)a->N * dD * dH * dW_ * Nout;
                splitk = splitk_fit(a, splitk, p.part_sz);
                p.part = (float*)a->ws;
            }
        }
        p.splitk = splitk;
        p.tm = (int)((Mmax + BM - 1) / BM); p.tn = (int)((Nout + BN - 1) / BN);
        dim3 grid((unsigned)(p.tm * p.tn), 1, (unsigned)(phases * splitk));
        if (wm == 2 && wn == 2) err = launch_fd<2, 2>(p, vec, grid, st);
        else if (wm == 2 && wn == 1) err = launch_fd<2, 1>(p, vec, grid, st);
        else if (wm == 1 && wn == 2) err = launch_fd<1, 2>(p, vec, grid, st);
        else err = launch_fd<1, 1>(p, vec, grid, st);
        if (splitk > 1 && err == hipSuccess) {
            splitk_fold(p.out, p.part, splitk, p.part_sz, a->beta, Nout, 0, 0, st);
            err = hipGetLastError();
        }
    } else if (a->mode == SAVP_CONV_WGRAD) {
        p.out = (float*)a->w;
        if (algo != 1) {
            int rc = SAVP_OK;
            if (conv_wgrad_patch_try(p, a, st, &rc)) return rc;
            if (algo == 2) return SAVP_EINVAL;
        }
        if (a->src_bf16 || a->out_bf16) return SAVP_EINVAL;
        WgPlan g;
        if (!wgrad_generic_plan(a, p.bf16 != 0, wm, wn, g)) return SAVP_EINVAL;
        wm = g.wm; wn = g.wn;
        const long long M = g.M, ktiles = g.ktiles;
        const bool va = g.va, vb = g.vb, wbf16 = g.wbf16;
        const int BM = 64 * wm, BN = 64 * wn;
        int splitk = g.splitk;
// ... 39 lines not shown
```

### video_prediction_amd/csrc/opts.h

```cpp
#pragma once

enum SavpOptId {
    OPT_CONV_RING = 0,
    OPT_S2DGRAD,
    OPT_THIN,
    OPT_WGP_CFG,
    OPT_WGP_SPLIT,
    OPT_INORM_MIN_HW,
    OPT_COLSUM_2STAGE,
    OPT_DENSE_LEGACY,
    OPT_CDNA_LEGACY,
    OPT_LSTM_FUSED,
    OPT_RING_DMA,
    OPT_LSTM_Q,
    OPT_RING_WWARM,
    OPT_WGP_DMA,
    OPT_RING_EARLY,
    OPT_GATE_KERNEL,
    OPT_GATE_ALT,
    OPT_GATE_CELL,
    OPT_GATE_WWARM,
    OPT_SPLITK_REDUCED,
    OPT_COUNT
};

int savp_opt(int id);
void savp_opt_count(int id);

#ifdef __HIPCC__
template <int BYTES>
__device__ __forceinline__ void kernarg_warm() {
    constexpr int LINES = (BYTES + 63) / 64;
    const unsigned long long ka = (unsigned long long)__builtin_amdgcn_kernarg_segment_ptr();
    unsigned t[LINES];
#pragma unroll
    for (int i = 0; i < LINES; ++i) asm volatile("s_load_dword %0, %1, %2" : "=&s"(t[i]) : "s"(ka), "n"(i * 64) : "memory");
    asm volatile("s_waitcnt lgkmcnt(0)" ::: "memory");
#pragma unroll
    for (int i = 0; i < LINES; ++i) asm volatile("" :: "s"(t[i]));
}
#endif
```

### video_prediction_amd/engine.py

```python
import math
import os
from collections import OrderedDict

import numpy as np
import torch

from . import kernels as K
from . import lib
from .variables import is_trainable


def _align4(n):
    return (n + 3) // 4 * 4


class Arena(object):

    def __init__(self, shapes, device):
        self.offsets = OrderedDict()
        off = 0
        for name, shape in shapes.items():
            n = int(np.prod(shape)) if len(shape) else 1
            self.offsets[name] = (off, n, tuple(shape))
            off += _align4(n)
# ... 143 lines not shown
            grp.fold64()
        return OrderedDict((n, self.grad(n).detach().cpu().numpy().copy()) for n in self.specs if self.group_of[n] != 'aux')


def same_pad_before(k, s, in_size):
    out = -(-in_size // s)
    total = max((out - 1) * s + k - in_size, 0)
    return total // 2


TRANSPOSED = ('up', 'deconv')


class ConvLayer(object):

    def __init__(self, store, kernel_name, bias_name, kind, ksize, stride, pad, sn_u=None, cx_pad=None, cy_pad=None):
        self.store = store
        self.kernel_name, self.bias_name, self.kind = kernel_name, bias_name, kind
        W = store[kernel_name]
        self.W = W
        self.dW = store.grad(kernel_name) if store.group_of[kernel_name] != 'aux' else None
        self.bias = store[bias_name] if bias_name else None
        self.dbias = store.grad(bias_name) if bias_name else None
        dev = W.device
        if kind == 'conv':
            self.cx, self.cy = W.shape[-2], W.shape[-1]
            self.wf = W
            self.dwf = None
            k3 = tuple(ksize)
        elif kind == 'pool':
            k, _, cin, cout = W.shape
            self.cx, self.cy = cin, cout
            self.wf = torch.empty(k + 1, k + 1, cin, cout, device=dev)
            self.dwf = torch.zeros_like(self.wf)
            k3 = (1, k + 1, k + 1)
        elif kind == 'up':
            k, _, cin, f = W.shape
            self.cx, self.cy = f, cin
            self.wf = torch.empty(k + 3, k + 3, f, cin, device=dev)
            self.dwf = torch.zeros_like(self.wf)
            k3 = (1, k + 3, k + 3)
        elif kind in ('down', 'deconv'):
            k, _, cx, cy = W.shape
            self.cx, self.cy = cx, cy
            self.wf = torch.empty(k + 1, k + 1, cx, cy, device=dev)
            self.dwf = torch.zeros_like(self.wf)
            k3 = (1, k + 1, k + 1)
        else:
            raise ValueError(kind)
        if len(k3) == 2:
            k3 = (1,) + tuple(k3)
        s3 = tuple(stride) if len(stride) == 3 else (1,) + tuple(stride)
        p3 = tuple(pad) if len(pad) == 3 else (0,) + tuple(pad)
        self.geom = K.ConvGeom(k3, s3, p3)
        self.taps = k3[0] * k3[1] * k3[2]
        self.cx0, self.cy0 = self.cx, self.cy
        self.padded = False
        if (cx_pad and cx_pad != self.cx) or (cy_pad and cy_pad != self.cy):
            if kind in ('up', 'deconv') or sn_u:
                raise NotImplementedError('channel padding for upsample / spectral-norm layers')
            self.padded = True
            self.cx, self.cy = cx_pad or self.cx, cy_pad or self.cy
            self.wfp = torch.zeros(self.taps, self.cx, self.cy, device=dev)
            self.dwfp = torch.zeros(self.taps, self.cx, self.cy, device=dev)
            self.dw_tmp = torch.empty(self.taps, self.cx0, self.cy0, device=dev)
            if self.bias is not None:
                self.bias_master, self.dbias_master = self.bias, self.dbias
                self.bias = torch.zeros(self.cy, device=dev)
                self.dbias = torch.zeros(self.cy, device=dev)
        self.wt = torch.empty(self.cy, self.taps * self.cx, device=dev)
        self.wd = torch.empty(self.cx, self.taps * self.cy, device=dev)
        self.wt16 = torch.empty(self.cy, self.taps * self.cx, device=dev, dtype=torch.bfloat16)
        self.wd16 = torch.empty(self.cx, self.taps * self.cy, device=dev, dtype=torch.bfloat16)
        self.sn_u_name = sn_u
        if sn_u:
            self.u = store[sn_u]
            kdim = W.numel() // self.cy
            self.sn_ws = torch.zeros(K.sn_ws_size(kdim, self.cy), device=dev)
            self.u_next = torch.empty_like(self.u)
            self.dwf = torch.zeros_like(W)
        self.need_wt = self.need_wd = True
        self.wfrag = None
        self.wfrag_il = None
        self.prof = None
        self.ktimer = None

    def sn_entry(self, update_u=False):
        return {'W': self.W, 'u': self.u.reshape(-1), 'ws': self.sn_ws, 'u_new': self.u_next.reshape(-1) if update_u else None}

    def sn_bwd_entry(self):
        return {'W': self.W, 'u': self.u.reshape(-1), 'ws': self.sn_ws, 'G': self.dwf, 'dW': self.dW, 'beta': 1}

    def prep(self, update_u=False, sn_done=False, defer_pack=None):
        scale = None
        if self.kind == 'pool':
            K.fold_pool(self.W, self.wf, self.W.shape[0])
        elif self.kind == 'up':
            k, _, cin, f = self.W.shape
            K.fold_bilinear(self.W, self.wf, k, cin, f)
        elif self.kind in ('down', 'deconv'):
            K.fold_embed(self.W, self.wf, self.W.shape[0])
        if self.sn_u_name:
            if not sn_done:
                K.sn_fwd(self.W, self.u.reshape(-1), self.sn_ws, self.u_next.reshape(-1) if update_u else None)
            scale = self.sn_ws[1:2]
        src = self.wf
        if self.padded:
            copy_view(self.wf.reshape(self.taps, self.cx0, self.cy0), [self.wfp[:, :self.cx0, :self.cy0]])
            if self.bias is not None:
                K.axpby(1.0, self.bias_master, 0.0, None, self.bias[:self.cy0])
            src = self.wfp
        b16 = K.PRECISION['value'] == 1
        entry = {'src': src, 'wt': self.wt if self.need_wt else None, 'wd': self.wd if self.need_wd else None, 'scale': scale,
                 'wt16': self.wt16 if (b16 and self.need_wt) else None, 'wd16': self.wd16 if (b16 and self.need_wd) else None}
        if defer_pack is not None:
            defer_pack.append(entry)
        else:
            K.pack_weights(**entry)
        if self.wfrag is not None and b16:
            K.pack_gate_weights(src, self.wfrag)
            if self.wfrag_il is not None:
                K.pack_gate_weights(src, self.wfrag_il, interleave=True)

    def enable_gate_pack(self, cell=False):
        if self.kind == 'conv' and not self.padded and not self.sn_u_name:
            n = K.gate_weights_elems(self.taps, self.cx, self.cy)
            if n:
                self.wfrag = torch.empty(n, device=self.W.device, dtype=torch.bfloat16)
                if cell and self.cy % 32 == 0:
                    self.wfrag_il = torch.empty(n, device=self.W.device, dtype=torch.bfloat16)

    def commit_u(self):
        if self.sn_u_name:
            self.u.copy_(self.u_next)

    def forward(self, x, y, beta=0, act=0, alpha=0.0, use_bias=True, stats=None, defer=False):
        b = self.bias if use_bias else None
        if self.kind == 'conv' and x.dim() == 2 and x.shape[0] <= 64 and not act and not beta and y.is_contiguous():
            if defer:
                return None
            K.dense_fwd(x, self.W.reshape(-1, self.cy), b, y, scale=self.sn_ws[1:2] if self.sn_u_name else None)
            return
        if defer:
            if self.ktimer is not None or self.prof is not None:
                return None
            if self.kind in TRANSPOSED:
                return K.conv(lib.CONV_DGRAD, self.geom, y, x, self.wd, bias=b, beta=beta, act=act, alpha=alpha, w16=self.wd16, stats=stats,
                              defer=True)
            return K.conv(lib.CONV_FPROP, self.geom, x, y, self.wt, bias=b, beta=beta, act=act, alpha=alpha, w16=self.wt16, stats=stats,
                          defer=True, w_frag=self.wfrag, w_frag_il=self.wfrag_il)
        if self.ktimer is not None:
            self.ktimer.arm()
        if self.prof is not None:
            e0, e1 = torch.cuda.Event(enable_timing=True), torch.cuda.Event(enable_timing=True)
            e0.record()
        if self.kind in TRANSPOSED:
            K.conv(lib.CONV_DGRAD, self.geom, y, x, self.wd, bias=b, beta=beta, act=act, alpha=alpha, w16=self.wd16, stats=stats)
        else:
            K.conv(lib.CONV_FPROP, self.geom, x, y, self.wt, bias=b, beta=beta, act=act, alpha=alpha, w16=self.wt16, stats=stats, w_frag=self.wfrag)
        if self.prof is not None:
            e1.record()
            self.prof.append((e0, e1))
        if self.ktimer is not None:
            self.ktimer.taken()

    def stats_ok(self, x, y):
        if K.PRECISION['value'] != 1:
            return False
        if self.kind in TRANSPOSED:
            return K.conv_stats_ok(lib.CONV_DGRAD, self.geom, y, x, self.wd, bias=self.bias, w16=self.wd16)
        return K.conv_stats_ok(lib.CONV_FPROP, self.geom, x, y, self.wt, bias=self.bias, w16=self.wt16)

    def backward_data(self, dy, dx, beta=0, act=0, alpha=0.0, aux=None, skip=None, norm_bwd=None, defer=False):
        if self.kind in TRANSPOSED:
            return K.conv(lib.CONV_FPROP, self.geom, dy, dx, self.wt, beta=beta, act=act, alpha=alpha, aux=aux, w16=self.wt16, dst_gap=skip,
                          norm_bwd=norm_bwd, defer=defer)
        return K.conv(lib.CONV_DGRAD, self.geom, dx, dy, self.wd, beta=beta, act=act, alpha=alpha, aux=aux, w16=self.wd16, dst_gap=skip,
                      norm_bwd=norm_bwd, defer=defer)

    def norm_bwd_ok(self, dy, dx, norm_bwd, skip=None):
        if K.PRECISION['value'] != 1:
            return False
        nb = dict(norm_bwd, ws=None)
        if self.kind in TRANSPOSED:
            return K.conv_stats_ok(lib.CONV_FPROP, self.geom, dy, dx, self.wt, w16=self.wt16, dst_gap=skip, norm_bwd=nb)
        return K.conv_stats_ok(lib.CONV_DGRAD, self.geom, dx, dy, self.wd, w16=self.wd16, dst_gap=skip, norm_bwd=nb)

    def backward_weights(self, x, dy, feeds_instance_norm=False):
        target = self.dwfp if self.padded else (self.dwf if self.dwf is not None else self.dW)
        if dy.dtype == torch.bfloat16 and self.dbias is not None and not feeds_instance_norm:
            raise NotImplementedError('bias gradient from a bf16 output gradient: only for a convolution in front of an instance norm '
                                      '(feeds_instance_norm=True), whose bias gradient is identically zero')
        db = None if (feeds_instance_norm and dy.dtype == torch.bfloat16) else self.dbias
        if self.kind in TRANSPOSED:
            K.conv(lib.CONV_WGRAD, self.geom, dy, x, target)
            if db is not None:
                K.colsum(dy, db)
        else:
            K.conv(lib.CONV_WGRAD, self.geom, x, dy, target, bias=db)

    def finish_weight_grad(self, sn_done=False):
        if self.padded:
            copy_view(self.dwfp[:, :self.cx0, :self.cy0], [self.dw_tmp])
            tgt = self.dwf if self.dwf is not None else self.dW
            K.axpby(1.0, self.dw_tmp.reshape(-1), 1.0, tgt.reshape(-1), tgt.reshape(-1))
            self.dwfp.zero_()
            if self.bias is not None:
                K.axpby(1.0, self.dbias[:self.cy0], 1.0, self.dbias_master, self.dbias_master)
                self.dbias.zero_()
        if self.dwf is None:
            return
        if self.sn_u_name:
            if not sn_done:
                K.sn_bwd(self.W, self.u.reshape(-1), self.sn_ws, self.dwf, self.dW, beta=1)
        elif self.kind == 'pool':
            K.fold_pool(self.dwf, self.dW, self.W.shape[0], adjoint=True)
        elif self.kind == 'up':
            k, _, cin, f = self.W.shape
            K.fold_bilinear(self.dwf, self.dW, k, cin, f, adjoint=True)
        elif self.kind in ('down', 'deconv'):
            K.fold_embed(self.dwf, self.dW, self.W.shape[0], adjoint=True)
        self.dwf.zero_()


class _TensorStore(object):

    def __init__(self, tensors, grads):
        self.t, self.g = tensors, grads
        self.group_of = {k: 'g' for k in tensors}

    def __getitem__(self, name):
        return self.t[name]

    def grad(self, name):
        return self.g[name]


def prep_layers(convs, **kw):
    if os.environ.get('SAVP_PACK_BATCH', '1') != '1':
        for c in convs:
            c.prep(**kw)
        return
    packs = []
    for c in convs:
        c.prep(defer_pack=packs, **kw)
    if packs:
        K.pack_weights_batch(packs)


class ConcatConv(object):

    def __init__(self, store, parts, ksize, stride, pad):
        self.parts = []
        off = 0
        W0 = store[parts[0][0]]
        self.lead = tuple(W0.shape[:-1])
        dev = W0.device
        for kname, bname in parts:
            W = store[kname]
            if tuple(W.shape[:-1]) != self.lead:
                raise ValueError('ConcatConv parts must share kernel size and input channels')
            cy = W.shape[-1]
            self.parts.append(dict(W=W, dW=store.grad(kname), b=store[bname], db=store.grad(bname), off=off, cy=cy))
            off += cy
        self.cy = off
        self.Wcat = torch.empty(self.lead + (off,), device=dev)
        self.dWcat = torch.zeros(self.lead + (off,), device=dev)
        self.bcat = torch.zeros(off, device=dev)
        self.dbcat = torch.zeros(off, device=dev)
# ... 75 lines not shown
```

### video_prediction_amd/kernels.py

```python
import ctypes

import torch

from . import debug as _debug
from . import lib
from .lib import (c_f32, c_i32, c_i64, c_vp, ptr)


def _nd(t):
    if t.stride(-1) != 1 and t.shape[-1] != 1:
        raise ValueError('channel stride must be 1')
    if t.dim() == 4:
        N, H, W, C = t.shape
        sn, sh, sw, _ = t.stride()
        return N, 1, H, W, C, sn, 0, sh, sw
    if t.dim() == 5:
        N, D, H, W, C = t.shape
        sn, sd, sh, sw, _ = t.stride()
        return N, D, H, W, C, sn, sd, sh, sw
    if t.dim() == 2:
        N, C = t.shape
        return N, 1, 1, 1, C, t.stride(0), 0, 0, 0
    raise ValueError('expected 2-D, 4-D or 5-D tensor')


class ConvGeom(object):

    def __init__(self, k, s=(1, 1, 1), p=(0, 0, 0)):
        if len(k) == 2:
            k, s, p = (1,) + tuple(k), (1,) + tuple(s), (0,) + tuple(p)
        self.k, self.s, self.p = tuple(k), tuple(s), tuple(p)

    def out_dims(self, D, H, W, pad_after):
        return tuple((i + pb + pa - k) // s + 1 for i, k, s, pb, pa in zip((D, H, W), self.k, self.s, self.p, pad_after))


PRECISION = {'value': 0}


def set_conv_precision(name):
    PRECISION['value'] = {'f32': 0, 'fp32': 0, 'bf16': 1}[name]


AUTOTUNE = {'enabled': False, 'cache': {}, 'log': [], 'dist': None, 'rejected': [], 'check_all': False}
CONV_CALL_LOG = None
INSITU = None


def save_tuning(path):
    import json
    with open(path, 'w') as f:
        json.dump({repr(k): list(v) for k, v in AUTOTUNE['cache'].items()}, f, indent=0, sort_keys=True)


def load_tuning(path):
    import ast
    import json
    with open(path) as f:
        d = json.load(f)
    for k, v in d.items():
        AUTOTUNE['cache'][ast.literal_eval(k)] = (int(v[0]), int(v[1]))
    sync_tuning_table()
    return len(d)


def set_tuning_group(dist_module, force=False):
    AUTOTUNE['dist'] = dist_module if (dist_module is not None and (dist_module.get_world_size() > 1 or force)) else None
    sync_tuning_table()


def sync_tuning_table():
    d = AUTOTUNE['dist']
    if d is None:
        return
    box = [dict(AUTOTUNE['cache']) if d.get_rank() == 0 else None]
    d.broadcast_object_list(box, src=0)
    AUTOTUNE['cache'].clear()
    AUTOTUNE['cache'].update(box[0])


def enable_autotune(flag=True):
    AUTOTUNE['enabled'] = bool(flag)


def _fill_conv_args(mode, geom, x, y, w, bias, beta, act, alpha, aux, splitk, tile, precision, w16=None, stats=None, dst_gap=None,
                    norm_bwd=None, w_frag=None, w_frag_il=None):
    a = lib.SavpConvArgs()
    a.mode = mode
    N, D, H, W, Cx, a.x_sn, a.x_sd, a.x_sh, a.x_sw = _nd(x)
    N2, Do, Ho, Wo, Cy, a.y_sn, a.y_sd, a.y_sh, a.y_sw = _nd(y)
    if N != N2:
        raise ValueError('batch mismatch %d vs %d' % (N, N2))
    a.N, a.D, a.H, a.W, a.Cx = N, D, H, W, Cx
    a.Do, a.Ho, a.Wo, a.Cy = Do, Ho, Wo, Cy
    if dst_gap is not None and dst_gap[1]:
        a.dst_gap_at, a.dst_gap = int(dst_gap[0]), int(dst_gap[1])
        if mode == lib.CONV_DGRAD:
            a.Cx = Cx - a.dst_gap
        elif mode == lib.CONV_FPROP:
            a.Cy = Cy - a.dst_gap
        else:
            raise ValueError('dst_gap: FPROP / DGRAD only')
    if norm_bwd is not None:
        nb = norm_bwd
        xv = view(nb['x'])
        a.nb_x, a.nb_x_sn, a.nb_x_sp = xv.p, xv.sn, xv.sp
        a.nb_mean, a.nb_rstd = nb['mean'].data_ptr(), nb['rstd'].data_ptr()
        a.nb_gamma, a.nb_beta = nb['gamma'].data_ptr(), nb['beta'].data_ptr()
        a.nb_ws = nb['ws'].data_ptr() if nb.get('ws') is not None else 16
        a.nb_c0, a.nb_nc = int(nb.get('c0', 0)), nb['x'].shape[-1]
        a.nb_act, a.nb_alpha = ACT_IDS[nb.get('act', 'relu')], float(nb.get('alpha', 0.0))
    a.kd, a.kh, a.kw = geom.k
    a.sd, a.sh, a.sw = geom.s
    a.pd, a.ph, a.pw = geom.p
    a.beta, a.act, a.alpha, a.splitk, a.tile = int(beta), int(act), float(alpha), int(splitk), int(tile)
    a.precision = PRECISION['value'] if precision is None else int(precision)
    a.x, a.y, a.w = x.data_ptr(), y.data_ptr(), w.data_ptr()
    a.bias = bias.data_ptr() if bias is not None else None
    a.aux = aux.data_ptr() if aux is not None else None
    a.w_bf16 = w16.data_ptr() if w16 is not None else None
    src, dst = (y, x) if mode == lib.CONV_DGRAD else (x, y)
    a.src_bf16 = int(src.dtype == torch.bfloat16)
    a.out_bf16 = int((y if mode == lib.CONV_WGRAD else dst).dtype == torch.bfloat16)
    a.stats = stats.data_ptr() if stats is not None else None
    a.w_frag = w_frag.data_ptr() if w_frag is not None else None
    a.w_frag_il = w_frag_il.data_ptr() if w_frag_il is not None else None
    taps = geom.k[0] * geom.k[1] * geom.k[2]
    if w.numel() != taps * Cx * Cy:
        raise ValueError('weight has %d elements, expected %d' % (w.numel(), taps * Cx * Cy))
    if aux is not None:
        dst = x if mode == lib.CONV_DGRAD else y
        if aux.stride() != dst.stride() or aux.shape != dst.shape:
            raise ValueError('aux must be addressed like the destination')
    return a


def _tune(a, mode, dst, w, return_all=False):
    if lib.get().savp_conv_special(ctypes.byref(a)):
        return [] if return_all else (0, 0)
    torch.cuda.synchronize()
    fn = lib.get().savp_conv
    st = lib.stream()
    tiles = (0x22, 0x21, 0x12, 0x11)
    if mode == lib.CONV_WGRAD:
        cands = [(t, sk) for t in tiles for sk in (0,)]
        scratch = torch.zeros_like(w)
        real_w, real_bias = a.w, a.bias
        a.w = scratch.data_ptr()
        a.bias = None
    else:
        splits = (1, 2, 4, 8) if a.act == 0 else (1,)
        algs = (0x300, 0x700) if (a.src_bf16 or a.out_bf16 or a.stats or a.nb_ws or a.dst_gap) else (0x100, 0x200, 0x600, 0x1200, 0x1600, 0x2200, 0x2600, 0x300, 0x700)
        if a.out_bf16 or a.stats:
            splits = (1,)
        cands = [(alg | t, sk) for alg in algs for t in tiles for sk in splits]
        cands += [(alg | 0x1000 | 0x11, sk) for alg in algs if (alg & 0x300) == 0x300 for sk in splits]
        real_dst, real_beta = (a.x if mode == lib.CONV_DGRAD else a.y), a.beta
        scratch = None
        real_stats = a.stats
        if a.stats:
            stats_scratch = torch.zeros(a.N * (a.Cx if mode == lib.CONV_DGRAD else a.Cy) * 2, device=dst.device, dtype=torch.float64)
            a.stats = stats_scratch.data_ptr()
        real_nb = a.nb_ws
        if a.nb_ws:
            nb_scratch = torch.zeros(a.N * a.nb_nc * 2, device=dst.device, dtype=torch.float64)
            a.nb_ws = nb_scratch.data_ptr()
        if a.beta:
            scratch = torch.empty_like(dst)
            if scratch.stride() != dst.stride():
                scratch = torch.empty(dst.untyped_storage().size() // 4, device=dst.device)
            if mode == lib.CONV_DGRAD:
                a.x = scratch.data_ptr()
            else:
                a.y = scratch.data_ptr()
            a.beta = 0
    best, best_t = None, 1e30
    every = []
    e0, e1 = torch.cuda.Event(enable_timing=True), torch.cuda.Event(enable_timing=True)
    for tile, sk in cands:
        a.tile, a.splitk = tile, sk
        a.ws, a.ws_bytes = None, 0
        if mode == lib.CONV_WGRAD or sk != 1:
            _conv_scratch(a, dst.device)
        if fn(st, ctypes.byref(a)) != 0:
            continue
        t = 1e30
        for _ in range(3):
            e0.record()
            for _ in range(4):
                fn(st, ctypes.byref(a))
            e1.record()
            e1.synchronize()
            t = min(t, e0.elapsed_time(e1))
        every.append((t, tile, sk))
        if t < best_t:
            best, best_t = (tile, sk), t
    bad = []
    if every and not return_all:
        check = sorted(every) if AUTOTUNE.get('check_all') else [e for e in every if (e[1], e[2]) == best]
        check = [e for e in check if (e[1], e[2]) != (0, 0)]
        if check:
            bad = _verify_candidates(a, mode, dst, w, [(t_, sk_) for _, t_, sk_ in check])
            if best in [b[0] for b in bad]:
                ok = [e for e in sorted(every) if (e[1], e[2]) not in [b[0] for b in bad]] if AUTOTUNE.get('check_all') else []
                best = (ok[0][1], ok[0][2]) if ok else (0, 0)
    if mode == lib.CONV_WGRAD:
        a.w, a.bias = real_w, real_bias
    else:
        a.beta = real_beta
        a.stats = real_stats
        a.nb_ws = real_nb
        if mode == lib.CONV_DGRAD:
            a.x = real_dst
        else:
            a.y = real_dst
    a.ws, a.ws_bytes = None, 0
    if return_all:
        return sorted(every)
    _tune.last_rejected = bad
    return best or (0, 0)


def _verify_candidates(a, mode, dst, w, cfgs):
    fn, st = lib.get().savp_conv, lib.stream()
    keep = (a.x, a.y, a.w, a.stats, a.nb_ws, a.tile, a.splitk, a.ws, a.ws_bytes, a.beta)
    if mode == lib.CONV_WGRAD:
        like, out_bf16 = w, False
    else:
        like, out_bf16 = dst, dst.dtype == torch.bfloat16
    ext = 1 + sum((n - 1) * s_ for n, s_ in zip(like.shape, like.stride()) if n > 0)
    nst = a.N * (a.Cx if mode == lib.CONV_DGRAD else a.Cy) * 2 if keep[3] else 0
    nnb = a.N * a.nb_nc * 2 if keep[4] else 0

    def run(cfg):
        out = torch.zeros(ext, device=like.device, dtype=like.dtype)
        sts = torch.zeros(max(nst, 1), device=like.device, dtype=torch.float64)
        nbs = torch.zeros(max(nnb, 1), device=like.device, dtype=torch.float64)
        if mode == lib.CONV_WGRAD:
            a.w = out.data_ptr()
        elif mode == lib.CONV_DGRAD:
            a.x = out.data_ptr()
        else:
            a.y = out.data_ptr()
        if nst:
            a.stats = sts.data_ptr()
        if nnb:
            a.nb_ws = nbs.data_ptr()
        a.tile, a.splitk = cfg
        a.ws, a.ws_bytes = None, 0
        if mode == lib.CONV_WGRAD or cfg[1] != 1:
            _conv_scratch(a, like.device)
        rc = fn(st, ctypes.byref(a))
        return rc, out, sts, nbs

    def differs(got, ref, tol):
        g, r = got.double(), ref.double()
        scale = float(r.abs().max())
        err = float((g - r).abs().max()) if g.numel() else 0.0
        if not (err <= tol * max(scale, 1e-30)):
            return 'max |diff| %.3g against max |ref| %.3g (tol %.1g)' % (err, scale, tol)
        return None

    bad = []
    try:
        rc, ref, ref_st, ref_nb = run((0, 0))
        if rc != 0:
            return []
        tol = 2e-2 if out_bf16 else (1e-2 if a.precision == 1 and mode == lib.CONV_WGRAD else 2e-4)
        for cfg in cfgs:
            rc, out, sts, nbs = run(cfg)
            why = 'rc %d' % rc if rc != 0 else (differs(out, ref, tol) or (nst and differs(sts, ref_st, 1e-3)) or (nnb and differs(nbs, ref_nb, 1e-3)))
            if why:
                bad.append((cfg, why))
    finally:
        a.x, a.y, a.w, a.stats, a.nb_ws, a.tile, a.splitk, a.ws, a.ws_bytes, a.beta = keep
    return bad


def _conv_scratch(a, device):
    need = lib.get().savp_conv_workspace_bytes(ctypes.byref(a))
    if need:
        ws = scratch(device, (need + 3) // 4)
        a.ws, a.ws_bytes = ws.data_ptr(), ws.numel() * 4


def conv(mode, geom, x, y, w, bias=None, beta=0, act=0, alpha=0.0, aux=None, splitk=0, tile=0, precision=None, w16=None, stats=None,
         dst_gap=None, norm_bwd=None, defer=False, w_frag=None, w_frag_il=None):
    lib.require_device(w, bias, aux)
    lib.require_stats(stats, (norm_bwd or {}).get('ws'))
    lib.require_device_any(x, y)
    a = _fill_conv_args(mode, geom, x, y, w, bias, beta, act, alpha, aux, splitk, tile, precision, w16, stats, dst_gap, norm_bwd, w_frag, w_frag_il)
    if AUTOTUNE['enabled'] and tile == 0 and splitk == 0 and not lib.get().savp_conv_special(ctypes.byref(a)):
        key = (mode, a.precision, a.N, a.D, a.H, a.W, a.Cx, a.Do, a.Ho, a.Wo, a.Cy, geom.k, geom.s, geom.p, a.act, a.beta,
               a.x_sw, a.y_sw, bias is not None, w16 is not None, a.src_bf16, a.out_bf16, stats is not None)
        if a.dst_gap:
            key = key + ((a.dst_gap_at, a.dst_gap),)
        if norm_bwd is not None:
            key = key + (('nb', a.nb_c0, a.nb_nc),)
        cfg = AUTOTUNE['cache'].get(key)
        if cfg is None:
            dst = x if mode == lib.CONV_DGRAD else y
            cfg = _tune(a, mode, dst, w)
            for bad_cfg, why in getattr(_tune, 'last_rejected', []):
                AUTOTUNE['rejected'].append((key, {'cfg': list(bad_cfg), 'why': why}))
            if AUTOTUNE['dist'] is not None:
                t = torch.tensor([int(cfg[0]), int(cfg[1])], dtype=torch.int32, device=dst.device)
                AUTOTUNE['dist'].broadcast(t, src=0)
                cfg = tuple(int(v) for v in t.tolist())
            AUTOTUNE['cache'][key] = cfg
            AUTOTUNE['log'].append((key, cfg))
        a.tile, a.splitk = cfg
        if INSITU is not None:
            if INSITU['mode'] == 'rank':
                if key in INSITU['targets'] and key not in INSITU['ranked']:
                    INSITU['ranked'][key] = _tune(a, mode, x if mode == lib.CONV_DGRAD else y, w, return_all=True)
                    a.tile, a.splitk = cfg
            elif INSITU['mode'] == 'all' or key in INSITU['targets']:
                if mode == lib.CONV_WGRAD or a.splitk != 1:
                    _conv_scratch(a, w.device)
                e0, e1 = torch.cuda.Event(enable_timing=True), torch.cuda.Event(enable_timing=True)
                e0.record()
                lib.check(lib.get().savp_conv(lib.stream(), ctypes.byref(a)), 'savp_conv')
                e1.record()
                INSITU['events'].append((key, e0, e1))
                return
    if mode == lib.CONV_WGRAD or a.splitk != 1:
        _conv_scratch(a, w.device)
    if CONV_CALL_LOG is not None:
        CONV_CALL_LOG.append((mode, a.N, a.D, a.H, a.W, a.Cx, a.Do, a.Ho, a.Wo, a.Cy, tuple(geom.k), tuple(geom.s), a.tile, a.splitk))
    if defer:
        return a
    rc = lib.get().savp_conv(lib.stream(), ctypes.byref(a))
    if rc:
        lib.check(rc, 'savp_conv(%s)' % describe_conv(a))


def describe_conv(a):
    return ('%s N=%d in=%dx%dx%dx%d out=%dx%dx%dx%d k=%dx%dx%d s=%dx%dx%d prec=%s x=%s%s y=%s%s tile=0x%x splitk=%d act=%d beta=%d bias=%d' %
            (('fprop', 'dgrad', 'wgrad')[a.mode], a.N, a.D, a.H, a.W, a.Cx, a.Do, a.Ho, a.Wo, a.Cy, a.kd, a.kh, a.kw, a.sd, a.sh, a.sw,
             'bf16' if a.precision == 1 else 'f32', 'bf16' if a.src_bf16 else 'f32', '/sw%d' % a.x_sw, 'bf16' if a.out_bf16 else 'f32',
             '/sw%d' % a.y_sw, a.tile, a.splitk, a.act, a.beta, 1 if a.bias else 0))


def conv_stats_ok(mode, geom, x, y, w, bias=None, w16=None, dst_gap=None, norm_bwd=None):
    a = _fill_conv_args(mode, geom, x, y, w, bias, 0, 0, 0.0, None, 0, 0, None, w16, None, dst_gap, norm_bwd)
    return bool(lib.get().savp_conv_stats_ok(ctypes.byref(a)))


ACT_IDS = {None: 0, 'none': 0, 'relu': 1, 'lrelu': 2, 'elu': 3}


def view(t, any_dtype=False):
    if any_dtype:
        lib.require_device_any(t)
    else:
        lib.require_device(t)
    if t.dim() < 3:
        t = t.reshape(t.shape[0], 1, t.shape[-1])
    if t.stride(-1) != 1 and t.shape[-1] != 1:
        raise ValueError('channel stride must be 1')
    sp = t.stride(-2)
    exp = sp
    for d in range(t.dim() - 2, 0, -1):
        if t.shape[d] != 1 and t.stride(d) != exp:
            raise ValueError('view is not pixel-linear: shape %s stride %s' % (tuple(t.shape), t.stride()))
        exp *= t.shape[d]
    v = lib.SavpView()
    v.p, v.sn, v.sp = t.data_ptr(), t.stride(0), sp
    return v


class _Acc64(object):

    def __init__(self, *tensors):
        self.pairs, self.out = [], []
        for t in tensors:
            if t is None:
                self.out.append(None)
            elif t.dtype == torch.float64:
                lib.require_stats(t)
                self.out.append(t)
            else:
                lib.require_device(t)
                d = torch.zeros(t.shape, dtype=torch.float64, device=t.device)
                self.pairs.append((t, d))
                self.out.append(d)

    def ptr(self, i):
        t = self.out[i]
        return ctypes.c_void_p(t.data_ptr()) if t is not None else ctypes.c_void_p(0)

    def addr(self, i):
        t = self.out[i]
        return t.data_ptr() if t is not None else None

    def finish(self, deferred=False):
        if deferred and self.pairs:
            raise TypeError('a deferred (fused) launch takes float64 accumulators (ParamGroup.grad64)')
        for t, d in self.pairs:
            t.add_(d.to(torch.float32))


def _hw(t):
    n = 1
    for d in t.shape[1:-1]:
        n *= d
    return n


def _set_views(arr, tensors, any_dtype=False):
    for i, t in enumerate(tensors):
        arr[i] = view(t, any_dtype)


def _bf16_mask(tensors):
    m = 0
    for i, t in enumerate(tensors):
        if t.dtype == torch.bfloat16:
            m |= 1 << i
        elif t.dtype != torch.float32:
            raise TypeError('expected float32 or bfloat16, got %s' % t.dtype)
    return m


class Scratch(object):

    def __init__(self, device):
        self.device, self.buf, self.retired = device, None, []
# ... 686 lines not shown
    acc.finish()


def reparam_bwd(mu, ls_raw, eps, dz, klw, dmu, dls_raw, klw_dev=None):
    rows = mu.numel() // mu.shape[-1]
    lib.check(_L().savp_reparam_bwd(lib.stream(), mu.numel(), rows, _p(mu), _p(ls_raw), _p(eps), _p(dz), float(klw), _p(dmu),
                                    _p(dls_raw), _p(klw_dev) if klw_dev is not None else None), 'savp_reparam_bwd')


def lp_loss(pred, target, weight, loss_out=None, dpred=None, p2=False):
    rows = pred.shape[0]
    row_len = pred[0].numel()
    assert pred[0].is_contiguous() and target[0].is_contiguous() and target.shape == pred.shape
    if dpred is not None:
        assert dpred.stride() == pred.stride()
    acc = _Acc64(loss_out)
    lib.check(_L().savp_lp_loss(lib.stream(), rows, row_len, pred.stride(0), target.stride(0), int(p2), _p(pred), _p(target),
                                float(weight), acc.addr(0), _p(dpred)), 'savp_lp_loss')
    acc.finish()


def tv_loss(flows, n_channels, s1, s2, weight, loss_out=None, dflows=None):
    lib.require_device_any(flows)
    assert flows.dtype == torch.float32 and flows.dim() == 4 and flows.stride(3) == 1 and flows.stride(1) == flows.shape[2] * flows.stride(2)
    if dflows is not None:
        assert dflows.stride() == flows.stride() and dflows.dtype == torch.float32
    lib.require_stats(loss_out)
    n, H, W, _ = flows.shape
    lib.check(_L().savp_tv_loss(lib.stream(), _p(flows), n, H, W, int(n_channels), flows.stride(0), flows.stride(2), float(s1), float(s2),
                                float(weight), _p(loss_out), _p(dflows)), 'savp_tv_loss')


def lsgan_loss(logits, label, weight, loss_out=None, dlogits=None, beta=0):
    acc = _Acc64(loss_out)
    lib.check(_L().savp_lsgan_loss(lib.stream(), logits.numel(), _p(logits), float(label), float(weight), acc.addr(0), _p(dlogits),
                                   int(beta)), 'savp_lsgan_loss')
    acc.finish()


def cosine_distance(f0, f1, weight, loss_out=None, df0=None, beta=0, eps=1e-10):
    assert f0.is_contiguous() and f1.is_contiguous()
    C = f0.shape[-1]
    acc = _Acc64(loss_out)
    lib.check(_L().savp_cosine_distance(lib.stream(), f0.numel() // C, C, _p(f0), _p(f1), float(weight), float(eps), acc.addr(0),
                                        _p(df0), int(beta)), 'savp_cosine_distance')
    acc.finish()


def pack_weights(src, wt=None, wd=None, scale=None, wt16=None, wd16=None):
    Cx, Cy = src.shape[-2], src.shape[-1]
    T = src.numel() // (Cx * Cy)
    lib.check(_L().savp_pack_weights(lib.stream(), _p(src), T, Cx, Cy, _p(scale), _p(wt), _p(wd), _p(wt16), _p(wd16)),
              'savp_pack_weights')


def pack_weights_batch(entries):
    for lo in range(0, len(entries), 32):
        part = entries[lo:lo + 32]
        arr = (lib.SavpPackItem * len(part))()
        for i, e in enumerate(part):
            src = e['src']
            lib.require_device(src)
            it = arr[i]
            it.src, it.scale = _p(src), _p(e.get('scale'))
            it.wt, it.wd, it.wt_bf16, it.wd_bf16 = _p(e.get('wt')), _p(e.get('wd')), _p(e.get('wt16')), _p(e.get('wd16'))
            it.Cx, it.Cy = src.shape[-2], src.shape[-1]
            it.T = src.numel() // (it.Cx * it.Cy)
        lib.check(_L().savp_pack_weights_batch(lib.stream(), len(part), arr), 'savp_pack_weights_batch')


def gate_weights_elems(taps, Cx, Cy):
    return int(lib.get().savp_gate_weights_bytes(int(taps), int(Cx), int(Cy))) // 2


def pack_gate_weights(src, out, interleave=False):
    lib.require_device(src)
    Cx, Cy = src.shape[-2], src.shape[-1]
    taps = src.numel() // (Cx * Cy)
    if out.dtype != torch.bfloat16 or out.numel() != gate_weights_elems(taps, Cx, Cy):
        raise ValueError('gate weight pack: expected %d bf16 elements' % gate_weights_elems(taps, Cx, Cy))
    lib.check(_L().savp_pack_gate_weights(lib.stream(), _p(src), taps, Cx, Cy, _p(out), int(bool(interleave))), 'savp_pack_gate_weights')


def fold_pool(inp, out, k, adjoint=False):
    C = (out.numel() if adjoint else inp.numel()) // (k * k)
    lib.check(_L().savp_fold_pool(lib.stream(), _p(inp), _p(out), k, C, int(adjoint)), 'savp_fold_pool')


def fold_embed(inp, out, k, adjoint=False):
    C = (out.numel() if adjoint else inp.numel()) // (k * k)
    if (inp.numel() if adjoint else out.numel()) != (k + 1) * (k + 1) * C:
        raise ValueError('fold_embed: %s <-> %s with k = %d' % (tuple(inp.shape), tuple(out.shape), k))
    lib.check(_L().savp_fold_embed(lib.stream(), _p(inp), _p(out), k, C, int(adjoint)), 'savp_fold_embed')


def fold_bilinear(inp, out, k, Cin, F, adjoint=False):
    lib.check(_L().savp_fold_bilinear(lib.stream(), _p(inp), _p(out), k, Cin, F, int(adjoint)), 'savp_fold_bilinear')


def sn_ws_size(K, C):
    return 8 + 2 * C + 2 * K + 2 * (C + 2)


def sn_fwd(W, u, ws, u_new=None):
    C = W.shape[-1]
    K = W.numel() // C
    lib.check(_L().savp_sn_fwd(lib.stream(), _p(W), K, C, _p(u), _p(ws), _p(u_new)), 'savp_sn_fwd')


def _sn_items(entries, bwd):
    arr = (lib.SavpSnItem * len(entries))()
    for i, e in enumerate(entries):
        W = e['W']
        C = W.shape[-1]
        arr[i].W, arr[i].K, arr[i].C = W.data_ptr(), W.numel() // C, C
        arr[i].u, arr[i].ws = e['u'].data_ptr(), e['ws'].data_ptr()
        arr[i].u_new = e['u_new'].data_ptr() if e.get('u_new') is not None else None
        if bwd:
            arr[i].G, arr[i].dW, arr[i].beta = e['G'].data_ptr(), e['dW'].data_ptr(), int(e.get('beta', 0))
    return arr


def sn_fwd_batch(entries):
    for lo in range(0, len(entries), 16):
        part = entries[lo:lo + 16]
        arr = _sn_items(part, False)
        lib.check(_L().savp_sn_fwd_batch(lib.stream(), len(part), arr), 'savp_sn_fwd_batch')


def sn_bwd_batch(entries):
    for lo in range(0, len(entries), 16):
        part = entries[lo:lo + 16]
        arr = _sn_items(part, True)
        lib.check(_L().savp_sn_bwd_batch(lib.stream(), len(part), arr), 'savp_sn_bwd_batch')


def sn_bwd(W, u, ws, G, dW, beta=0):
    C = W.shape[-1]
    K = W.numel() // C
    lib.check(_L().savp_sn_bwd(lib.stream(), _p(W), K, C, _p(u), _p(ws), _p(G), _p(dW), int(beta)), 'savp_sn_bwd')


def dense_fwd(x, W, bias, out, scale=None):
    M, Kd = x.shape
    C = W.shape[-1]
    assert out.is_contiguous() and x.stride(1) == 1 and W.is_contiguous()
    ws = scratch(x.device, 64 * M * C)
    lib.check(_L().savp_dense_fwd(lib.stream(), _p(x), x.stride(0), M, Kd, C, _p(W), _p(bias), _p(scale), _p(out), _p(ws), ws.numel()),
              'savp_dense_fwd')


def _warp_args(img, flows, K_):
    a = lib.SavpWarpArgs()
    a.N, a.H, a.W, a.C = img.shape
    a.K = K_
    a.img = view(img)
    assert flows.is_contiguous() and flows.shape[-1] == 2 * K_
    a.flows = _p(flows)
    return a


def image_warp_fwd(img, flows, out, K_):
    a = _warp_args(img, flows, K_)
    a.out = view(out)
    lib.check(_L().savp_image_warp_fwd(lib.stream(), ctypes.byref(a)), 'savp_image_warp_fwd')

# ... 382 lines not shown
```

### video_prediction_amd/lib.py

```python
import ctypes
import os

import torch

from . import debug as _debug

_HERE = os.path.dirname(os.path.abspath(__file__))
LIB_PATH = os.environ.get('SAVP_LIB') or os.path.join(_HERE, 'libsavp_hip.so')

c_i32, c_i64, c_f32, c_vp = ctypes.c_int32, ctypes.c_int64, ctypes.c_float, ctypes.c_void_p

CONV_FPROP, CONV_DGRAD, CONV_WGRAD = 0, 1, 2
ACT_NONE, ACT_LRELU, ACT_SIGMOID, ACT_DLRELU_FROM_OUT = 0, 1, 2, 3


class SavpConvArgs(ctypes.Structure):
    _fields_ = [
        ('mode', c_i32),
        ('N', c_i32), ('D', c_i32), ('H', c_i32), ('W', c_i32), ('Cx', c_i32),
        ('Do', c_i32), ('Ho', c_i32), ('Wo', c_i32), ('Cy', c_i32),
        ('kd', c_i32), ('kh', c_i32), ('kw', c_i32),
        ('sd', c_i32), ('sh', c_i32), ('sw', c_i32),
        ('pd', c_i32), ('ph', c_i32), ('pw', c_i32),
        ('beta', c_i32), ('act', c_i32), ('alpha', c_f32), ('splitk', c_i32), ('tile', c_i32), ('precision', c_i32),
        ('x', c_vp), ('x_sn', c_i64), ('x_sd', c_i64), ('x_sh', c_i64), ('x_sw', c_i64),
        ('y', c_vp), ('y_sn', c_i64), ('y_sd', c_i64), ('y_sh', c_i64), ('y_sw', c_i64),
        ('w', c_vp), ('bias', c_vp), ('aux', c_vp), ('w_bf16', c_vp),
        ('src_bf16', c_i32), ('out_bf16', c_i32), ('stats', c_vp),
        ('ws', c_vp), ('ws_bytes', c_i64),
        ('dst_gap_at', c_i32), ('dst_gap', c_i32),
        ('nb_x', c_vp), ('nb_x_sn', c_i64), ('nb_x_sp', c_i64), ('nb_mean', c_vp), ('nb_rstd', c_vp), ('nb_gamma', c_vp), ('nb_beta', c_vp),
        ('nb_ws', c_vp), ('nb_c0', c_i32), ('nb_nc', c_i32), ('nb_act', c_i32), ('nb_alpha', c_f32),
        ('w_frag', c_vp), ('w_frag_il', c_vp),
    ]


class SavpJpegArgs(ctypes.Structure):
    _fields_ = [
        ('N', c_i32), ('width', c_i32), ('height', c_i32), ('components', c_i32),
        ('h', c_i32 * 3), ('v', c_i32 * 3), ('blocks_w', c_i32 * 3), ('blocks_h', c_i32 * 3), ('block_offset', c_i32 * 3),
        ('total_blocks', c_i32), ('out_h', c_i32), ('out_w', c_i32),
        ('coef', c_vp), ('qtab', c_vp), ('window', c_vp), ('out', c_vp), ('ws', c_vp), ('ws_bytes', c_i64),
    ]


_lib = None


def get():
    global _lib
    if _lib is None:
        if not os.path.exists(LIB_PATH):
            raise RuntimeError(
                'libsavp_hip.so not found at %s -- build it first (python -c "import __graft_entry__ as g; g.build()"). '
                'video_prediction_amd has no non-HIP fallback.' % LIB_PATH)
        lib = ctypes.CDLL(LIB_PATH)
        lib.savp_version.restype = ctypes.c_char_p
        _declare(lib)
        _lib = lib
        _forward_env_options(lib)
    if _debug.POISON['lds']:
        return _LdsPoisonProxy(_lib)
    return _lib


def get_raw():
    lib = get()
    return lib._lib if isinstance(lib, _LdsPoisonProxy) else lib


class _LdsPoisonProxy(object):

    def __init__(self, lib):
        self._lib = lib

    def __getattr__(self, name):
        fn = getattr(self._lib, name)
        at = getattr(fn, 'argtypes', None)
        if not name.startswith('savp_') or name.startswith(('savp_debug_', 'savp_prof_')) or not at or at[0] is not c_vp or \
                name in ('savp_allreduce_bucket',):
            return fn
        poison = self._lib.savp_debug_poison_lds

        def call(st, *args):
            poison(st, _debug.NAN_WORD, None)
            _debug.COUNTS['lds'] += 1
            return fn(st, *args)
        return call


OPTION_NAMES = ('conv_ring', 's2dgrad', 'thin', 'wgp_cfg', 'wgp_split', 'inorm_min_hw', 'colsum_2stage', 'dense_legacy', 'cdna_legacy',
                'lstm_fused', 'ring_dma', 'lstm_q', 'ring_wwarm', 'wgp_dma', 'ring_early', 'gate_kernel', 'gate_alt', 'gate_cell', 'gate_wwarm', 'splitk_reduced')


def set_option(name, value):
    check(get().savp_set_option(name.encode(), int(value)), 'savp_set_option(%s)' % name)


def get_option(name):
    v = c_i32()
    check(get().savp_get_option(name.encode(), ctypes.byref(v)), 'savp_get_option(%s)' % name)
    return v.value


def _forward_env_options(lib):
    for name in OPTION_NAMES:
        v = os.environ.get('SAVP_' + name.upper())
        if v is not None:
            check(lib.savp_set_option(name.encode(), int(v)), 'savp_set_option(%s)' % name)


EXPORTS = {}


def _sig(lib, name, argtypes, restype=c_i32):
    try:
        fn = getattr(lib, name)
    except AttributeError:
        if os.environ.get('SAVP_LIB'):
            return None
        raise
    fn.argtypes = argtypes
    fn.restype = restype
    EXPORTS[name] = fn
    return fn


def _declare(lib):
    P = ctypes.POINTER
    _sig(lib, 'savp_conv', [c_vp, P(SavpConvArgs)])
    _sig(lib, 'savp_conv_workspace_bytes', [P(SavpConvArgs)], restype=c_i64)
    _sig(lib, 'savp_conv_special', [P(SavpConvArgs)])
    _sig(lib, 'savp_gate_weights_bytes', [c_i32, c_i32, c_i32], restype=c_i64)
    _sig(lib, 'savp_conv_stats_ok', [P(SavpConvArgs)])
    _sig(lib, 'savp_set_option', [ctypes.c_char_p, c_i32])
    _sig(lib, 'savp_get_option', [ctypes.c_char_p, P(c_i32)])
    _sig(lib, 'savp_allreduce_bucket', [c_vp, c_vp, c_vp, c_i64])
    _sig(lib, 'savp_tiled_z_weff', [c_vp, c_vp, c_i32, c_i32, c_i32, c_i32, c_i32, c_i32, c_i32, c_i32, c_vp])
    _sig(lib, 'savp_tiled_z_grad', [c_vp, c_vp, c_i32, c_i64, c_i32, c_i32, c_i32, c_vp, c_i32, c_vp, c_i32, c_vp, c_i64])
    _sig(lib, 'savp_tiled_z_workspace_bytes', [c_i64, c_i32], restype=c_i64)
    _sig(lib, 'savp_eval_fold_ws_floats', [c_i32, c_i32, c_i32, c_i32], restype=c_i64)
    _sig(lib, 'savp_jpeg_workspace_bytes', [P(SavpJpegArgs)], restype=c_i64)
    for name, argtypes in _EXTRA_SIGS.items():
        _sig(lib, name, argtypes)


_EXTRA_SIGS = {}


def register(name, argtypes):
    _EXTRA_SIGS[name] = argtypes
    if _lib is not None:
        _sig(_lib, name, argtypes)


def source_id():
    import hashlib
    h = hashlib.sha256()
    root = os.path.dirname(_HERE)
    files = []
    for d, pat in ((os.path.join(_HERE, 'csrc'), ('.hip', '.h')), (os.path.join(root, 'include'), ('.h',)), (_HERE, ('.json',))):
        for f in sorted(os.listdir(d)):
            if f.endswith(pat) and (d != _HERE or f.startswith('tuning_gfx950_')):
                files.append(os.path.join(d, f))
    for f in files:
        h.update(os.path.basename(f).encode())
        with open(f, 'rb') as fh:
            h.update(fh.read())
    return h.hexdigest()[:16]


def stream():
    return ctypes.c_void_p(torch.cuda.current_stream().cuda_stream)


# ... 196 lines not shown
register('savp_fold_embed', [c_vp, c_vp, c_vp, c_i32, c_i64, c_i32])
register('savp_fold_bilinear', [c_vp, c_vp, c_vp, c_i32, c_i32, c_i32, c_i32])
class SavpPackItem(ctypes.Structure):
    _fields_ = [('src', c_vp), ('scale', c_vp), ('wt', c_vp), ('wd', c_vp), ('wt_bf16', c_vp), ('wd_bf16', c_vp), ('T', c_i64),
                ('Cx', c_i32), ('Cy', c_i32)]


register('savp_pack_weights_batch', [c_vp, c_i32, ctypes.POINTER(SavpPackItem)])


class SavpSnItem(ctypes.Structure):
    _fields_ = [('W', c_vp), ('K', c_i64), ('C', c_i32), ('u', c_vp), ('ws', c_vp), ('u_new', c_vp), ('G', c_vp), ('dW', c_vp),
                ('beta', c_i32)]


register('savp_sn_fwd_batch', [c_vp, c_i32, ctypes.POINTER(SavpSnItem)])
register('savp_sn_bwd_batch', [c_vp, c_i32, ctypes.POINTER(SavpSnItem)])
register('savp_sn_fwd', [c_vp, c_vp, c_i64, c_i32, c_vp, c_vp, c_vp])
register('savp_sn_bwd', [c_vp, c_vp, c_i64, c_i32, c_vp, c_vp, c_vp, c_vp, c_i32])
register('savp_dense_fwd', [c_vp, c_vp, c_i64, c_i32, c_i64, c_i32, c_vp, c_vp, c_vp, c_vp, c_vp, c_i64])


class SavpWarpArgs(ctypes.Structure):
    _fields_ = [('N', c_i32), ('H', c_i32), ('W', c_i32), ('C', c_i32), ('K', c_i32), ('img', SavpView), ('flows', c_vp),
                ('out', SavpView), ('dout', SavpView), ('dflows', c_vp), ('dimg', c_vp)]


class SavpDnaArgs(ctypes.Structure):
    _fields_ = [('N', c_i32), ('H', c_i32), ('W', c_i32), ('C', c_i32), ('K', c_i32), ('kh', c_i32), ('kw', c_i32),
                ('img', SavpView), ('raw', c_vp), ('kern', c_vp), ('out', SavpView), ('dout', SavpView), ('draw', c_vp),
                ('dimg', SavpView), ('dimg_beta', c_i32)]


MAX_SOURCES = 4


class SavpCdnaMultiArgs(ctypes.Structure):
    _fields_ = [
        ('N', c_i32), ('H', c_i32), ('W', c_i32), ('C', c_i32), ('K', c_i32), ('kh', c_i32), ('kw', c_i32), ('nsrc', c_i32),
        ('img', SavpView * MAX_SOURCES), ('kern', c_vp), ('out', SavpView), ('dout', SavpView),
        ('dimg', SavpView * MAX_SOURCES), ('dimg_beta', c_i32 * MAX_SOURCES), ('dkern', c_vp),
    ]


class SavpWarpMultiArgs(ctypes.Structure):
    _fields_ = [('N', c_i32), ('H', c_i32), ('W', c_i32), ('C', c_i32), ('K', c_i32), ('nsrc', c_i32),
                ('img', SavpView * MAX_SOURCES), ('flows', c_vp), ('out', SavpView), ('dout', SavpView), ('dflows', c_vp),
                ('dimg', SavpView * MAX_SOURCES), ('dimg_beta', c_i32 * MAX_SOURCES)]


class SavpDnaMultiArgs(ctypes.Structure):
    _fields_ = [('N', c_i32), ('H', c_i32), ('W', c_i32), ('C', c_i32), ('K', c_i32), ('kh', c_i32), ('kw', c_i32), ('nsrc', c_i32),
                ('img', SavpView * MAX_SOURCES), ('raw', c_vp), ('kern', c_vp), ('out', SavpView), ('dout', SavpView), ('draw', c_vp),
                ('dimg', SavpView * MAX_SOURCES), ('dimg_beta', c_i32 * MAX_SOURCES)]


register('savp_cdna_apply_multi_fwd', [c_vp, ctypes.POINTER(SavpCdnaMultiArgs)])
register('savp_cdna_apply_multi_bwd', [c_vp, ctypes.POINTER(SavpCdnaMultiArgs)])
register('savp_image_warp_multi_fwd', [c_vp, ctypes.POINTER(SavpWarpMultiArgs)])
register('savp_image_warp_multi_bwd', [c_vp, ctypes.POINTER(SavpWarpMultiArgs)])
register('savp_dna_apply_multi_fwd', [c_vp, ctypes.POINTER(SavpDnaMultiArgs)])
register('savp_dna_apply_multi_bwd', [c_vp, ctypes.POINTER(SavpDnaMultiArgs)])
register('savp_image_warp_fwd', [c_vp, ctypes.POINTER(SavpWarpArgs)])
register('savp_image_warp_bwd', [c_vp, ctypes.POINTER(SavpWarpArgs)])
register('savp_dna_apply_fwd', [c_vp, ctypes.POINTER(SavpDnaArgs)])
register('savp_dna_apply_bwd', [c_vp, ctypes.POINTER(SavpDnaArgs)])


class SavpGruArgs(ctypes.Structure):
    _fields_ = [('N', c_i32), ('HW', c_i32), ('F', c_i32), ('eps', c_f32), ('pre', c_vp), ('h', SavpView),
                ('gamma', c_vp), ('beta', c_vp), ('mean', c_vp), ('rstd', c_vp), ('u', c_vp), ('rh', SavpView),
                ('nout', c_i32), ('out', SavpView * 4), ('ndy', c_i32), ('dy', SavpView * 4), ('dpre', c_vp), ('du', c_vp),
                ('dh', SavpView), ('drh', SavpView), ('dgamma', c_vp), ('dbeta', c_vp)]


for _n in ('savp_convgru_gates_fwd', 'savp_convgru_out_fwd', 'savp_convgru_out_bwd', 'savp_convgru_gates_bwd'):
    register(_n, [c_vp, ctypes.POINTER(SavpGruArgs)])
register('savp_gan_loss', [c_vp, c_i32, c_i32, c_vp, c_f32, c_f32, c_vp, c_vp, c_i32])
register('savp_fold_f64', [c_vp, c_vp, c_i64, c_vp, c_vp])
register('savp_tv_loss', [c_vp, c_vp, c_i32, c_i32, c_i32, c_i32, c_i64, c_i64, c_f32, c_f32, c_f32, c_vp, c_vp])
register('savp_state_pred_fwd', [c_vp, c_i32, c_i32, c_i32, c_i32] + [c_vp] * 7)
register('savp_state_pred_bwd', [c_vp, c_i32, c_i32, c_i32, c_i32] + [c_vp] * 6)
register('savp_pack_gate_weights', [c_vp, c_vp, c_i32, c_i32, c_i32, c_vp, c_i32])
register('savp_debug_poison_lds', [c_vp, ctypes.c_uint32, c_vp])
register('savp_debug_fill_u32', [c_vp, c_vp, c_i64, ctypes.c_uint32])
register('savp_debug_probe_lds', [c_vp, ctypes.c_uint32, c_vp])
```

### video_prediction_amd/models/savp_cell.py

```python
import os

import torch

from .. import kernels as K
from .. import lib
from ..engine import ConcatConv, ConvLayer, same_pad_before, copy_view, add_views, prep_layers
from ..variables import ACTIVATIONS, NORM_SCOPES, down_scope, layer_specs, num_masks, up_scope

CONV_STATS = os.environ.get('SAVP_CONV_STATS', '1') == '1'
FUSED_ENTRIES = os.environ.get('SAVP_FUSED_ENTRIES', '1') == '1'
NORM_BWD_STATS = os.environ.get('SAVP_NORM_BWD_STATS', '1') == '1'
EPS_IN = 1e-6


def check_norm_layers(hp):
    if hp.conv_rnn not in ('lstm', 'gru'):
        raise NotImplementedError("conv_rnn=%r" % hp.conv_rnn)
    if hp.norm_layer not in ('instance', 'layer'):
        raise NotImplementedError("norm_layer=%r: the HIP path covers 'instance' and 'layer'" % hp.norm_layer)
    if hp.conv_rnn_norm_layer not in ('instance', 'layer', 'none'):
        raise NotImplementedError("conv_rnn_norm_layer=%r: the HIP path covers 'instance', 'layer' and 'none'" % hp.conv_rnn_norm_layer)
    layer = 'layer' in (hp.norm_layer, hp.conv_rnn_norm_layer)
    if layer and not hp.use_tile_concat:
        raise NotImplementedError("use_tile_concat=False with norm_layer=%r, conv_rnn_norm_layer=%r: the untiled latent is only "
# ... 144 lines not shown
        if cw > 32:
            raise NotImplementedError('actions + states wider than 32 (csrc/state_pred.hip keeps them in registers)')
        tile = bool(hp.use_tile_concat)
        zr = zw if (hp.where_add == 'all' and tile) else 0
        g = train
        self.act16 = bool(K.PRECISION['value'] == 1 and hp.conv_rnn == 'lstm' and os.environ.get('SAVP_BF16_CONVIO', '1') == '1')
        a16 = torch.bfloat16 if self.act16 else torch.float32
        enc_specs, dec_specs = layer_specs(hp.ngf, H, W)
        self.ne, self.nd = len(enc_specs), len(dec_specs)

        self.layers = []
        h_, w_ = H, W
        prev_f = None
        for i, (f, use_rnn) in enumerate(enc_specs + dec_specs):
            L = {'f': f, 'rnn': use_rnn, 'idx': i, 'dec': i >= self.ne}
            s = prefix + 'h%d/' % i
            j_dec = i - len(enc_specs)
            zc = zw if (tile and (hp.where_add == 'all' or (hp.where_add == 'input' and i == 0) or
                                  (hp.where_add == 'middle' and j_dec == 0))) else 0
            L['zc'], L['zr'] = zc, zr
            if i < self.ne:
                cx = 2 * C if i == 0 else prev_f
                k = 5 if i == 0 else 3
                L['in'] = Act((T1, N, h_, w_, ceil8(cx + zc)), dev, grad=g,
                              dtype=a16 if i > 0 else torch.float32)
                L['zoff_in'] = cx
                L['conv'] = ConvLayer(store, s + self.down_op + '/kernel', s + self.down_op + '/bias',
                                      'pool' if self.down_op == 'conv_pool2d' else 'down', (k, k), (2, 2),
                                      (same_pad_before(k + 1, 2, h_), same_pad_before(k + 1, 2, w_)),
                                      cx_pad=ceil8(cx + zc))
                h_, w_ = h_ // 2, w_ // 2
            else:
                j = i - self.ne
                skip = 0 if j == 0 else self.layers[self.ne - j - 1]['f']
                cx = prev_f + skip
                L['in'] = Act((T1, N, h_, w_, cx + zc), dev, grad=g, dtype=a16 if (cx + zc) % 8 == 0 else torch.float32)
                L['zoff_in'] = cx
                L['skip_off'] = prev_f
                h_, w_ = h_ * 2, w_ * 2
                if self.up_op == 'deconv2d':
                    L['conv'] = ConvLayer(store, s + 'deconv2d/kernel', s + 'deconv2d/bias', 'deconv', (3, 3), (2, 2),
                                          (same_pad_before(4, 2, h_), same_pad_before(4, 2, w_)))
                else:
                    L['conv'] = ConvLayer(store, s + 'upsample_conv2d/kernel', s + 'upsample_conv2d/bias', 'up', (3, 3), (2, 2),
                                          (same_pad_before(6, 2, h_), same_pad_before(6, 2, w_)))
            L['hw'] = (h_, w_)
            pre16 = f % 8 == 0 and (i < self.ne or L['in'].v.dtype == torch.bfloat16 or not self.act16)
            L['pre'] = Act((T1, N, h_, w_, f), dev, grad=g, grad_dtype=a16 if pre16 else torch.float32)
            L['norm'] = self._norm(s, f, bias=L['conv'].bias_name)
            if use_rnn and self.abl_rnn:
                r = prefix + 'conv_h%d/' % i
                L['a'] = Act((T1, N, h_, w_, ceil4(f + zr)), dev, grad=g, dtype=a16 if ceil4(f + zr) % 8 == 0 else torch.float32)
                L['pre2'] = Act((T1, N, h_, w_, f), dev, grad=g, grad_dtype=a16 if f % 8 == 0 else torch.float32)
                L['rconv'] = ConvLayer(store, r + 'conv2d/kernel', r + 'conv2d/bias', 'conv', (5, 5), (1, 1), (2, 2), cx_pad=ceil4(f + zr))
                L['n2'] = self._norm(r, f, bias=r + 'conv2d/bias')
            elif use_rnn and hp.conv_rnn == 'gru':
                r = prefix + 'gru_h%d/conv2dgru_cell/' % i
                L['cin1'] = f + zr + f
                L['a'] = Act((T1, N, h_, w_, f + zr + 2 * f), dev, grad=g)
                L['gates'] = Act((T1, N, h_, w_, 2 * f), dev, grad=g)
                L['cand'] = Act((T1, N, h_, w_, f), dev, grad=g)
                L['u'] = torch.empty(T1, N, h_, w_, f, device=dev)
                L['du'] = torch.empty(N, h_, w_, f, device=dev) if g else None
                L['dh_tmp'] = torch.empty(N, h_, w_, f, device=dev) if g else None
                L['rconv'] = ConvLayer(store, r + 'gates/kernel', None, 'conv', (5, 5), (1, 1), (2, 2))
                L['cconv'] = ConvLayer(store, r + 'candidate/kernel', None, 'conv', (5, 5), (1, 1), (2, 2))
                L['n1'] = Norm(store, r + 'gates/reset_update/', T1, N, 2 * f, dev)
                L['n2'] = Norm(store, r + 'candidate/state/', T1, N, f, dev)
            elif use_rnn:
                r = prefix + 'lstm_h%d/basic_conv2dlstm_cell/' % i
                L['fused'] = (K.PRECISION['value'] == 1 and os.environ.get('SAVP_FUSED_CELL', '1') == '1' and not self.cell_plain and
                              not self.cell_ln and
                              h_ % 8 == 0 and w_ % 8 == 0 and 16 <= f <= 256 and (f & (f - 1)) == 0 and (f + zr + f) % 8 == 0)
                a_dt = torch.bfloat16 if (L['fused'] and os.environ.get('SAVP_BF16_ACT', '1') == '1') else torch.float32
                L['a'] = Act((T1, N, h_, w_, f + zr + f), dev, grad=g, dtype=a_dt)
                dg_dt = torch.bfloat16 if (L['fused'] and g and os.environ.get('SAVP_BF16_DGATES', '1') == '1') else torch.float32
                L['gates'] = Act((T1, N, h_, w_, 4 * f), dev, grad=g, dtype=torch.bfloat16 if L['fused'] else torch.float32,
                                 grad_dtype=dg_dt)
                L['dg_raw'] = torch.empty(N, h_, w_, 4 * f, device=dev) if dg_dt == torch.bfloat16 else None
                L['c'] = Act((T1, N, h_, w_, f), dev, grad=False)
                L['dc'] = [torch.empty(N, h_, w_, f, device=dev), torch.empty(N, h_, w_, f, device=dev)] if g else None
                L['rconv'] = ConvLayer(store, r + 'kernel', (r + 'bias') if self.cell_plain else None, 'conv', (5, 5), (1, 1), (2, 2))
                if not self.cell_plain and not self.cell_ln:
                    L['rconv'].enable_gate_pack(cell=bool(L['fused']) and h_ * w_ <= 256)
                if self.cell_ln:
                    L['gn4'] = ConcatNorm([Norm(store, r + nm + '/', T1, N, f, dev, groups=1) for nm in ('input', 'transform', 'forget', 'output')],
                                          T1, N, dev)
                    L['nS'] = Norm(store, r + 'state/', T1, N, f, dev, groups=1)
                    L['gnv'] = Act((T1, N, h_, w_, 4 * f), dev, grad=g)
                    L['cpre'] = Act((T1, N, h_, w_, f), dev, grad=g)
                    L['dcn'] = torch.empty(N, h_, w_, f, device=dev) if g else None
                elif not self.cell_plain:
                    L['n1'] = Norm(store, r + 'input_transform_forget_output/', T1, N, 4 * f, dev)
                    L['n2'] = Norm(store, r + 'state/', T1, N, f, dev)
                if self.out_norm:
                    L['h_raw'] = Act((T1, N, h_, w_, f), dev, grad=g)
                    L['onorm'] = self._norm(prefix + 'lstm_h%d/' % i, f, hp.conv_rnn_norm_layer)
                L['zless'] = bool(g and zr and not cw and L['fused'] and os.environ.get('SAVP_ZLESS_DGRAD', '1') == '1' and
                                  K.tiled_z_ok(h_, w_, 4 * f, zr, L['rconv'].geom))
                if L['zless']:
                    L['weff'] = torch.empty(25, 4 * f, K.tiled_z_pad(zr), device=dev)
            else:
                L['out'] = None
            self.layers.append(L)
            prev_f = f
        nl = len(self.layers)
        last = self.layers[-1]
        ngf = hp.ngf
        self.M = M = num_masks(hp)
        self.L = hp.last_frames
        self.nk = nk = hp.last_frames * hp.num_transformed_images
        self.nti = hp.num_transformed_images
        kh, kw = hp.kernel_size
        self.kh, self.kw = kh, kw

        self.tf = hp.transformation
        self.h_last = Act((T1, N, H, W, last['f']), dev, grad=g, dtype=a16 if last['f'] % 8 == 0 else torch.float32)
        tf_convs = []
        if self.tf == 'cdna':
            sh_, sw_ = H // 2 ** self.ne, W // 2 ** self.ne
            small_f = self.layers[self.ne - 1]['f']
            self.hsmall = Act((T1, N, sh_, sw_, small_f), dev, grad=g)
            self.cdna_dense = ConvLayer(store, prefix + 'cdna_kernels/dense/kernel', prefix + 'cdna_kernels/dense/bias', 'conv',
                                        (1, 1), (1, 1), (0, 0))
            self.cdna_raw = Act((T1, N, kh * kw * nk), dev, grad=g)
            self.cdna_kern = Act((T1, N, kh * kw, nk), dev, grad=False)
            self.cdna_dkern = torch.zeros(N, kh * kw, nk, device=dev, dtype=torch.float64) if g else None
            tf_convs = [self.cdna_dense]
        else:
            hs, os_, cy = (('h%d_flow/' % nl, 'flows/', 2 * nk) if self.tf == 'flow' else
                           ('h%d_dna_kernel/' % nl, 'dna_kernels/', kh * kw * nk))
            s = prefix + hs
            self.tf_conv = ConvLayer(store, s + 'conv2d/kernel', s + 'conv2d/bias', 'conv', (3, 3), (1, 1), (1, 1))
            self.tf_pre = Act((T1, N, H, W, ngf), dev, grad=g)
            self.tf_norm = self._norm(s, ngf, bias=s + 'conv2d/bias')
            self.tf_h = Act((T1, N, H, W, ngf), dev, grad=g)
            self.tf_out = ConvLayer(store, prefix + os_ + 'conv2d/kernel', prefix + os_ + 'conv2d/bias', 'conv', (3, 3), (1, 1),
                                    (1, 1), cy_pad=ceil4(cy))
            self.tf_cy = ceil4(cy)
            self.tf_raw = Act((T1, N, H, W, self.tf_cy), dev, grad=g)
            if self.tf == 'dna':
                if self.tf_cy != cy:
                    raise NotImplementedError('dna with kh*kw*nk not a multiple of 4')
                self.dna_kern = torch.empty(T1, N, H, W, cy, device=dev)
            tf_convs = [self.tf_conv, self.tf_out]
        self.merge_heads = os.environ.get('SAVP_MERGE_HEADS', '1') == '1' and ngf % 4 == 0
        sep = not self.merge_heads
        self.scratch = bool(hp.generate_scratch_image)
        self.dep_mask = bool(hp.dependent_mask)
        self.Cs = Cs = ceil4(C)
        if self.scratch:
            s = prefix + 'h%d_scratch/' % nl
            self.scratch_conv = ConvLayer(store, s + 'conv2d/kernel', s + 'conv2d/bias', 'conv', (3, 3), (1, 1), (1, 1))
            self.scratch_pre = Act((T1, N, H, W, ngf), dev, grad=g) if sep else None
            self.scratch_norm = self._norm(s, ngf, bias=s + 'conv2d/bias')
            self.scratch_h = Act((T1, N, H, W, ngf), dev, grad=g)
            s = prefix + 'scratch_image/'
            self.scratch_out = ConvLayer(store, s + 'conv2d/kernel', s + 'conv2d/bias', 'conv', (3, 3), (1, 1), (1, 1), cy_pad=Cs)
            self.dscratch_pre = torch.empty(T1, N, H, W, Cs, device=dev) if g else None
        s = prefix + 'h%d_masks/' % nl
        self.masks_conv = ConvLayer(store, s + 'conv2d/kernel', s + 'conv2d/bias', 'conv', (3, 3), (1, 1), (1, 1))
        self.masks_pre = Act((T1, N, H, W, ngf), dev, grad=g) if sep else None
        self.masks_norm = self._norm(s, ngf, bias=s + 'conv2d/bias')
        cf = hp.context_frames
        self.bgs = [('prev',)] if hp.prev_image_background else []
        if hp.context_images_background:
            self.bgs += [('fixed', k) for k in range(cf)]
        else:
            self.bgs += ([('fixed', 0)] if hp.first_image_background else []) + ([('fixed', cf - 1)] if hp.last_image_background else []) + \
                        ([('last_context',)] if hp.last_context_image_background else [])
        nb = len(self.bgs)
        assert M == nk + nb + int(self.scratch)
        if M < 2:
            raise NotImplementedError('a single transformed image (mask == 1 everywhere, savp_model.py:636-637)')
        self.Cmask = Cmask = ceil8(ngf + M * C + ((Cs - C) if self.scratch else 0))
        self.Ml = Ml = ceil4(M)
        self.maskin = Act((T1, N, H, W, Cmask), dev, grad=g)
        self.o_cdna = ngf
        self.o_bg = [ngf + (nk + i) * C for i in range(nb)]
        self.o_prev = self.o_bg[self.bgs.index(('prev',))] if ('prev',) in self.bgs else None
        self.o_scratch = ngf + (nk + nb) * C
        s = prefix + 'masks/'
        self.mask_cin = Cmask if self.dep_mask else ngf
        self.masks_out = ConvLayer(store, s + 'conv2d/kernel', s + 'conv2d/bias', 'conv', (3, 3), (1, 1), (1, 1),
# ... 634 lines not shown
```

Baseline: 10480.

## Add gate-conv data-gradient kernel with fused norm-backward stats epilogue

Extends the packed-weight gate convolution kernel with a DGRAD variant for the ConvLSTM recurrent 5x5 conv backward pass. Weights are pre-packed flipped and transposed into MFMA fragment order, with an optional channel gap. The epilogue writes dx and accumulates instance-norm backward sums (with activation gradient) into the double workspace via atomics. This is meant to replace the generic igemm dgrad plus a separate stats pass, at the cost of extra packing work, more template instantiations and shape restrictions.

```diff
diff --git a/include/savp_hip.h b/include/savp_hip.h
--- a/include/savp_hip.h
+++ b/include/savp_hip.h
@@ -59,6 +59,7 @@
     int32_t nb_c0, nb_nc, nb_act; float nb_alpha;
     const void* w_frag;
     const void* w_frag_il;
+    const void* w_frag_d;
 } SavpConvArgs;
 
 int savp_conv(void* stream, const SavpConvArgs* args);
@@ -425,6 +426,10 @@
 
 int64_t savp_gate_weights_bytes(int32_t taps, int32_t Cx, int32_t Cy);
 int savp_pack_gate_weights(void* stream, const float* src, int32_t taps, int32_t Cx, int32_t Cy, void* out, int32_t interleave);
+int savp_pack_gate_weights_dgrad(void* stream, const float* src, int32_t taps, int32_t Cx, int32_t Cy, int32_t gap_at, int32_t gap, void* out);
+int savp_gate_pack_fwd_ok(int32_t S, int32_t Cx, int32_t Cy);
+int savp_gate_pack_cell_ok(int32_t S, int32_t Cx, int32_t Cy);
+int savp_gate_pack_dgrad_ok(int32_t S, int32_t Cx, int32_t Cy, int32_t gap_at, int32_t gap);
 
 int savp_debug_poison_lds(void* stream, uint32_t pattern, void* sink);
 int savp_debug_fill_u32(void* stream, void* p, int64_t words, uint32_t pattern);
diff --git a/video_prediction_amd/csrc/common.hip b/video_prediction_amd/csrc/common.hip
--- a/video_prediction_amd/csrc/common.hip
+++ b/video_prediction_amd/csrc/common.hip
@@ -34,7 +34,7 @@
 
 static struct { const char* name; int value; } g_opts[OPT_COUNT] = {
     {"conv_ring", 0}, {"s2dgrad", 1}, {"thin", 1}, {"wgp_cfg", 0}, {"wgp_split", 0}, {"inorm_min_hw", 64}, {"colsum_2stage", 1},
-    {"dense_legacy", 0}, {"cdna_legacy", 0}, {"lstm_fused", 1}, {"ring_dma", 1}, {"lstm_q", 0}, {"ring_wwarm", 1}, {"wgp_dma", 1}, {"ring_early", 1}, {"gate_kernel", 1}, {"gate_alt", 0}, {"gate_cell", 1}, {"gate_wwarm", 1}, {"splitk_reduced", 0},
+    {"dense_legacy", 0}, {"cdna_legacy", 0}, {"lstm_fused", 1}, {"ring_dma", 1}, {"lstm_q", 0}, {"ring_wwarm", 1}, {"wgp_dma", 1}, {"ring_early", 1}, {"gate_kernel", 1}, {"gate_alt", 0}, {"gate_cell", 1}, {"gate_wwarm", 1}, {"gate_dgrad", 1}, {"splitk_reduced", 0},
 };
 int savp_opt(int id) { return g_opts[id].value; }
 void savp_opt_count(int id) { ++g_opts[id].value; }
diff --git a/video_prediction_amd/csrc/conv_common.h b/video_prediction_amd/csrc/conv_common.h
--- a/video_prediction_amd/csrc/conv_common.h
+++ b/video_prediction_amd/csrc/conv_common.h
@@ -150,5 +150,7 @@
 bool conv_ring_try(ConvP& p, const SavpConvArgs* a, int wm, int wn, hipStream_t st, int* rc, bool dry = false);
 bool conv_gate_applies(const SavpConvArgs* a);
 bool conv_gate_try(const SavpConvArgs* a, hipStream_t st, int* rc);
+bool conv_gate_dgrad_applies(const SavpConvArgs* a);
+bool conv_gate_dgrad_try(const SavpConvArgs* a, hipStream_t st, int* rc);
 struct SavpConvLstmCellArgs;
 bool conv_gate_cell_try(const SavpConvLstmCellArgs* c, hipStream_t st, int* rc);
diff --git a/video_prediction_amd/csrc/conv_gate.hip b/video_prediction_amd/csrc/conv_gate.hip
--- a/video_prediction_amd/csrc/conv_gate.hip
+++ b/video_prediction_amd/csrc/conv_gate.hip
@@ -20,6 +20,11 @@
     float* c_new;
     int nh; void* h[4]; long long h_sn[4], h_sp[4]; int h16;
     float *mean1, *rstd1, *mean2, *rstd2;
+    float* dx; long long dx_sn; int dx_sp;
+    int gap_at, gap;
+    const float* nb_x; long long nb_x_sn; int nb_x_sp;
+    const float *nb_mean, *nb_rstd, *nb_gamma, *nb_beta;
+    double* nb_ws; int nb_c0, nb_nc, nb_act; float nb_alpha;
 };
 
 __device__ __attribute__((aligned(16))) unsigned g_gate_zero[4] = {0u, 0u, 0u, 0u};
@@ -97,7 +102,7 @@
     }
 }
 
-template <int S, int CIN, int TM, int TN, int NWN, bool CELL = false>
+template <int S, int CIN, int TM, int TN, int NWN, bool CELL = false, bool DGRAD = false>
 __global__ __launch_bounds__(256, (2 * GateCfg<S, CIN, TM, TN, NWN>::LDSB <= 160 * 1024 ? 2 : 1)) void conv_gate_kernel(GateP p) {
     GT(0);
     using G = GateCfg<S, CIN, TM, TN, NWN>;
@@ -202,6 +207,33 @@
         for (int j = 0; j < TN; ++j)
 #pragma unroll
             for (int r = 0; r < 16; ++r) acc[i][j][r] = 0.f;
+
+    constexpr int DTMF = DGRAD ? TM / KSPLIT : 1;
+    static_assert(!DGRAD || (TN == 1 && !CELL && 32 * DTMF <= G::TR * G::TC), "DGRAD epilogue: one column block per wave, a wave's finished rows inside one image");
+    [[maybe_unused]] float dxv[DTMF][16];
+    [[maybe_unused]] float dmu = 0.f, drs = 0.f, dga = 0.f, dbe = 0.f;
+    [[maybe_unused]] bool nb_in = false;
+    [[maybe_unused]] int dfin = 0, dn = 0;
+    [[maybe_unused]] const int dcol = n0 + nw * G::NCW + l31;
+    if constexpr (DGRAD) {
+        dfin = KSPLIT == 4 ? (kq == 0 ? 0 : (kq == 2 ? TM / 4 : (kq == 1 ? TM / 2 : TM / 2 + TM / 4))) : (kq ? TM / 2 : 0);
+        dn = img0 + (dfin * 32) / (G::TR * G::TC);
+        const int cb0 = n0 + nw * G::NCW - p.nb_c0;
+        nb_in = p.nb_ws && cb0 >= 0 && cb0 < p.nb_nc;
+        if (nb_in) {
+            const int cc = dcol - p.nb_c0, nn = min(dn, p.N - 1);
+            dmu = p.nb_mean[(long long)nn * p.nb_nc + cc]; drs = p.nb_rstd[(long long)nn * p.nb_nc + cc];
+            dga = p.nb_gamma[cc]; dbe = p.nb_beta[cc];
+            const float* __restrict__ xp = p.nb_x + (long long)nn * p.nb_x_sn + cc;
+#pragma unroll
+            for (int i = 0; i < DTMF; ++i)
+#pragma unroll
+                for (int r = 0; r < 16; ++r) {
+                    const int rr = ((dfin + i) * 32 + (r & 3) + 8 * (r >> 2) + 4 * khalf) % (G::TR * G::TC);
+                    dxv[i][r] = xp[((ty0 + rr / G::TC) * S + tx0 + rr % G::TC) * p.nb_x_sp];
+                }
+        }
+    }
 
     GT(2);
     asm volatile("s_waitcnt vmcnt(0)" ::: "memory");
@@ -484,6 +516,62 @@
         return;
     }
 
+    if constexpr (DGRAD) {
+        float* dstat = reinterpret_cast<float*>(gsm);
+        const int pcol = dcol + (dcol >= p.gap_at ? p.gap : 0);
+        const bool live = dn < p.N;
+        float* __restrict__ db = p.dx + (long long)min(dn, p.N - 1) * p.dx_sn + pcol;
+        auto dfinish = [&](auto fin_c) {
+            constexpr int FIN = decltype(fin_c)::value;
+            float sm = 0.f, q = 0.f;
+#pragma unroll
+            for (int i = 0; i < DTMF; ++i)
+#pragma unroll
+                for (int r = 0; r < 16; ++r) {
+                    const float v = acc[FIN + i][0][r];
+                    if (nb_in) {
+                        const float xh = (dxv[i][r] - dmu) * drs;
+                        const float y = xh * dga + dbe;
+                        const float gr = p.nb_act == 1 ? (y > 0.f ? 1.f : 0.f) : (p.nb_act == 2 ? (y > 0.f ? 1.f : p.nb_alpha) : 1.f);
+                        const float d = v * gr;
+                        sm += d; q += d * xh;
+                    }
+                    const int rr = ((FIN + i) * 32 + (r & 3) + 8 * (r >> 2)) % (G::TR * G::TC) + 4 * khalf;
+                    if (live) db[((ty0 + rr / G::TC) * S + tx0 + rr % G::TC) * p.dx_sp] = v;
+                }
+            sm += __shfl_xor(sm, 32); q += __shfl_xor(q, 32);
+            if (p.nb_ws && khalf == 0) { dstat[(kq * NC + nw * G::NCW + l31) * 2] = sm; dstat[(kq * NC + nw * G::NCW + l31) * 2 + 1] = q; }
+        };
+        if constexpr (KSPLIT == 4) {
+            if (!odd && !hi) dfinish(IC0{});
+            else if (!odd && hi) dfinish(ICQ{});
+            else if (odd && !hi) dfinish(ICH{});
+            else dfinish(ICHQ{});
+        } else {
+            if (!odd) dfinish(IC0{}); else dfinish(ICH{});
+        }
+        GT(6);
+        if (p.nb_ws) {
+            __syncthreads();
+            constexpr int WPI = KSPLIT / G::NI;
+            for (int i = tid; i < G::NI * NC * 2; i += 256) {
+                const int im = i / (NC * 2), rem = i - im * (NC * 2);
+                const int n = img0 + im, cc = n0 + (rem >> 1) - p.nb_c0;
+                if (n >= p.N || cc < 0 || cc >= p.nb_nc) continue;
+                float t = 0.f;
+#pragma unroll
+                for (int o = 0; o < WPI; ++o) {
+                    const int ord = im * WPI + o;
+                    const int q_ = KSPLIT == 4 ? (((ord & 1) << 1) | (ord >> 1)) : ord;
+                    t += dstat[q_ * NC * 2 + rem];
+                }
+                unsafeAtomicAdd(p.nb_ws + ((long long)n * p.nb_nc + cc) * 2 + (rem & 1), (double)t);
+            }
+        }
+        GT(7);
+        return;
+    }
+
     float* stat = reinterpret_cast<float*>(gsm + (4 * G::XB > G::STGB ? 4 * G::XB : G::STGB));
     unsigned* T = reinterpret_cast<unsigned*>(gsm);
     constexpr int TMF = TM / KSPLIT;
@@ -601,20 +689,55 @@
     return hipGetLastError() == hipSuccess ? SAVP_OK : SAVP_ELAUNCH;
 }
 
-template <int S, int CIN, int TM, int TN, int NWN, bool CELL = false>
+__global__ __launch_bounds__(256) void pack_gate_weights_dgrad_kernel(const float* __restrict__ src, int taps, int Cx, int Cy, int ncol, int gap_at, int gap,
+                                                                      uint4* __restrict__ out) {
+    const int C8 = Cy >> 3, nch = taps * C8, KS = (nch + 1) >> 1;
+    const long long total = (long long)(ncol >> 5) * KS * 64;
+    for (long long t = total + (long long)blockIdx.x * 256 + threadIdx.x; t < total + GATE_PACK_PAD_KSTEPS * 64; t += (long long)gridDim.x * 256)
+        out[t] = make_uint4(0u, 0u, 0u, 0u);
+    for (long long t = (long long)blockIdx.x * 256 + threadIdx.x; t < total; t += (long long)gridDim.x * 256) {
+        const int lane = (int)(t & 63);
+        const long long r = t >> 6;
+        const int ks = (int)(r % KS), cb = (int)(r / KS);
+        const int c = 2 * ks + (lane >> 5);
+        typedef __bf16 bf16x2 __attribute__((ext_vector_type(2)));
+        unsigned w[4] = {0u, 0u, 0u, 0u};
+        if (c < nch) {
+            const int tap = c / C8, ch = c - tap * C8;
+            const int col = cb * 32 + (lane & 31), pc = col + (col >= gap_at ? gap : 0);
+            const float* s = src + ((long long)(taps - 1 - tap) * Cx + pc) * Cy + ch * 8;
+#pragma unroll
+            for (int j = 0; j < 4; ++j) w[j] = __builtin_bit_cast(unsigned, bf16x2{(__bf16)s[2 * j], (__bf16)s[2 * j + 1]});
+        }
+        out[t] = make_uint4(w[0], w[1], w[2], w[3]);
+    }
+}
+
+extern "C" int savp_pack_gate_weights_dgrad(void* stream, const float* src, int32_t taps, int32_t Cx, int32_t Cy, int32_t gap_at, int32_t gap, void* out) {
+    if (gap < 0 || gap_at < 0 || (gap && gap_at + gap > Cx)) return SAVP_EINVAL;
+    const int ncol = Cx - gap;
+    if (!src || !out || !savp_gate_weights_bytes(taps, Cy, ncol) || (((uintptr_t)out) & 15)) return SAVP_EINVAL;
+    const long long total = savp_gate_weights_bytes(taps, Cy, ncol) / 16 - GATE_PACK_PAD_KSTEPS * 64;
+    unsigned nb = (unsigned)((total + 255) / 256);
+    if (nb > 4096) nb = 4096;
+    hipLaunchKernelGGL(pack_gate_weights_dgrad_kernel, dim3(nb), dim3(256), 0, (hipStream_t)stream, src, taps, Cx, Cy, ncol, gap ? gap_at : 0x7fffffff, gap, (uint4*)out);
+    return hipGetLastError() == hipSuccess ? SAVP_OK : SAVP_ELAUNCH;
+}
+
+template <int S, int CIN, int TM, int TN, int NWN, bool CELL = false, bool DGRAD = false>
 static hipError_t launch_gate(const GateP& p, hipStream_t st) {
     using G = GateCfg<S, CIN, TM, TN, NWN>;
     static bool attr = false;
     if (!attr) {
-        hipFuncSetAttribute((const void*)conv_gate_kernel<S, CIN, TM, TN, NWN, CELL>, hipFuncAttributeMaxDynamicSharedMemorySize, G::LDSB);
+        hipFuncSetAttribute((const void*)conv_gate_kernel<S, CIN, TM, TN, NWN, CELL, DGRAD>, hipFuncAttributeMaxDynamicSharedMemorySize, G::LDSB);
         attr = true;
     }
     const dim3 grid((unsigned)(p.mtiles * p.ntiles));
     if (g_savp_prof_start) {
-        hipExtLaunchKernelGGL((conv_gate_kernel<S, CIN, TM, TN, NWN, CELL>), grid, dim3(256), G::LDSB, st, g_savp_prof_start, g_savp_prof_stop, 0, p);
+        hipExtLaunchKernelGGL((conv_gate_kernel<S, CIN, TM, TN, NWN, CELL, DGRAD>), grid, dim3(256), G::LDSB, st, g_savp_prof_start, g_savp_prof_stop, 0, p);
         g_savp_prof_start = g_savp_prof_stop = nullptr;
     } else {
-        hipLaunchKernelGGL((conv_gate_kernel<S, CIN, TM, TN, NWN, CELL>), grid, dim3(256), G::LDSB, st, p);
+        hipLaunchKernelGGL((conv_gate_kernel<S, CIN, TM, TN, NWN, CELL, DGRAD>), grid, dim3(256), G::LDSB, st, p);
     }
     return hipGetLastError();
 }
@@ -720,3 +843,86 @@
     *rc = err == hipSuccess ? SAVP_OK : SAVP_ELAUNCH;
     return true;
 }
+
+#define GATE_DGRAD_SHAPES(X)                                                                                              \
+    X(32, 128, 8, 1, 1, 0) X(16, 256, 4, 1, 1, 0)                                                                         \
+    X(32, 128, 4, 1, 2, 16)
+
+static bool gate_dgrad_shape_ok(int S, int cred, int ncol) {
+#define X(S_, C_, TM_, TN_, NWN_, ALT_) if (ALT_ == 0 && S == S_ && cred == C_ && ncol % GateCfg<S_, C_, TM_, TN_, NWN_>::NC == 0) return true;
+    GATE_DGRAD_SHAPES(X)
+#undef X
+    return false;
+}
+
+bool conv_gate_dgrad_applies(const SavpConvArgs* a) {
+    if (!savp_opt(OPT_GATE_KERNEL) || !savp_opt(OPT_GATE_DGRAD)) return false;
+    if (!(a->mode == SAVP_CONV_DGRAD && a->precision == SAVP_PREC_BF16 && a->src_bf16 && !a->out_bf16 && a->w_frag_d && !a->bias && !a->aux &&
+          a->act == SAVP_ACT_NONE && !a->beta && !a->stats && a->splitk <= 1))
+        return false;
+    if (!(a->D == 1 && a->Do == 1 && a->kd == 1 && a->kh == 5 && a->kw == 5 && a->sd == 1 && a->sh == 1 && a->sw == 1 && a->pd == 0 && a->ph == 2 &&
+          a->pw == 2 && a->H == a->W && a->Ho == a->H && a->Wo == a->W && a->N >= 1))
+        return false;
+    if (!(a->y_sw == a->Cy && a->y_sh == (long long)a->W * a->Cy && a->y_sn == (long long)a->H * a->W * a->Cy && aligned16(a->y) && aligned16(a->w_frag_d)))
+        return false;
+    if (!(a->x_sw >= 1 && a->x_sh == (long long)a->W * a->x_sw && a->x_sw * (long long)a->H * a->W < (1ll << 31) && !(((uintptr_t)a->x) & 3))) return false;
+    if (a->dst_gap && (a->dst_gap < 0 || a->dst_gap_at < 0 || (a->dst_gap_at & 31))) return false;
+    if (a->nb_ws) {
+        if (a->nb_c0 < 0 || a->nb_nc < 32 || (a->nb_c0 & 31) || (a->nb_nc & 31) || a->nb_c0 + a->nb_nc > a->Cx || a->nb_act < 0 || a->nb_act > 2 ||
+            (((uintptr_t)a->nb_ws) & 7) || a->nb_x_sp < 1 || a->nb_x_sp * (long long)a->H * a->W >= (1ll << 31))
+            return false;
+    }
+    return gate_dgrad_shape_ok(a->H, a->Cy, a->Cx);
+}
+
+bool conv_gate_dgrad_try(const SavpConvArgs* a, hipStream_t st, int* rc) {
+    if (!conv_gate_dgrad_applies(a)) return false;
+    static const void* zero_of[64] = {nullptr};
+    int dev_ord = 0;
+    if (hipGetDevice(&dev_ord) != hipSuccess || dev_ord < 0 || dev_ord >= 64) dev_ord = 0;
+    if (!zero_of[dev_ord] && hipGetSymbolAddress((void**)&zero_of[dev_ord], HIP_SYMBOL(g_gate_zero)) != hipSuccess) { *rc = SAVP_ELAUNCH; return true; }
+    GateP p = {};
+    p.x = (const unsigned short*)a->y; p.wfrag = (const uint4*)a->w_frag_d; p.y = nullptr; p.stats = nullptr;
+    p.zero16 = zero_of[dev_ord]; p.N = a->N; p.Cy = a->Cx; p.wwarm = savp_opt(OPT_GATE_WWARM);
+    p.dx = (float*)a->x; p.dx_sn = a->x_sn; p.dx_sp = (int)a->x_sw;
+    p.gap_at = a->dst_gap ? a->dst_gap_at : 0x7fffffff; p.gap = a->dst_gap;
+    p.nb_ws = (double*)a->nb_ws;
+    if (a->nb_ws) {
+        p.nb_x = a->nb_x; p.nb_x_sn = a->nb_x_sn; p.nb_x_sp = (int)a->nb_x_sp; p.nb_mean = a->nb_mean; p.nb_rstd = a->nb_rstd;
+        p.nb_gamma = a->nb_gamma; p.nb_beta = a->nb_beta; p.nb_c0 = a->nb_c0; p.nb_nc = a->nb_nc; p.nb_act = a->nb_act; p.nb_alpha = a->nb_alpha;
+    }
+    hipError_t err = hipErrorInvalidValue;
+    const int alt = savp_opt(OPT_GATE_ALT);
+    bool done = false;
+#define X(S_, C_, TM_, TN_, NWN_, ALT_)                                                                  \
+    if (!done && a->H == S_ && a->Cy == C_ && a->Cx % GateCfg<S_, C_, TM_, TN_, NWN_>::NC == 0 && (want ? (ALT_ & want) != 0 : ALT_ == 0)) {   \
+        using G = GateCfg<S_, C_, TM_, TN_, NWN_>;                                                       \
+        p.mtiles = G::NI == 1 ? a->N * G::TPI : (a->N + G::NI - 1) / G::NI; p.ntiles = a->Cx / G::NC;    \
+        err = launch_gate<S_, C_, TM_, TN_, NWN_, false, true>(p, st);                                   \
+        done = true;                                                                                     \
+    }
+    { const int want = alt; GATE_DGRAD_SHAPES(X) }
+    { const int want = 0; GATE_DGRAD_SHAPES(X) }
+#undef X
+    *rc = err == hipSuccess ? SAVP_OK : SAVP_ELAUNCH;
+    return true;
+}
+
+extern "C" int savp_gate_pack_fwd_ok(int32_t S, int32_t Cx, int32_t Cy) {
+    if (Cy < 128 || (Cy & 127)) return 0;
+#define X(S_, C_, TM_, TN_, NWN_, ALT_) if (S == S_ && Cx == C_) return 1;
+    GATE_SHAPES(X)
+#undef X
+    return 0;
+}
+extern "C" int savp_gate_pack_cell_ok(int32_t S, int32_t Cx, int32_t Cy) {
+    if (Cy < 128 || (Cy & 127)) return 0;
+#define X(S_, C_, TM_) if (S == S_ && Cx == C_) return 1;
+    GATE_CELL_SHAPES(X)
+#undef X
+    return 0;
+}
+extern "C" int savp_gate_pack_dgrad_ok(int32_t S, int32_t Cx, int32_t Cy, int32_t gap_at, int32_t gap) {
+    if (gap < 0 || gap_at < 0 || (gap && ((gap_at & 31) || gap_at + gap > Cx)) || Cx - gap < 32) return 0;
+    return gate_dgrad_shape_ok(S, Cy, Cx - gap) ? 1 : 0;
+}
diff --git a/video_prediction_amd/csrc/conv_igemm.hip b/video_prediction_amd/csrc/conv_igemm.hip
--- a/video_prediction_amd/csrc/conv_igemm.hip
+++ b/video_prediction_amd/csrc/conv_igemm.hip
@@ -775,7 +775,7 @@
 }
 
 extern "C" int savp_conv_special(const SavpConvArgs* a) {
-    if (a && conv_gate_applies(a)) return 1;
+    if (a && (conv_gate_applies(a) || conv_gate_dgrad_applies(a))) return 1;
     if (!a || ((a->tile >> 8) & 3) != 0) return 0;
     return (conv_thin_applies(a) || conv_s2dgrad_applies(a) || conv_gate_applies(a)) ? 1 : 0;
 }
@@ -783,6 +783,7 @@
 extern "C" int savp_conv_stats_ok(const SavpConvArgs* a) {
     if (!a || (a->mode != SAVP_CONV_FPROP && a->mode != SAVP_CONV_DGRAD) || a->precision != SAVP_PREC_BF16) return 0;
     if (((a->tile >> 8) & 3) == 0 && (conv_thin_applies(a) || conv_s2dgrad_applies(a))) return 0;
+    if (a->nb_ws && conv_gate_dgrad_applies(a)) return 1;
     const bool dg = a->mode == SAVP_CONV_DGRAD;
     const int Cred = dg ? a->Cy : a->Cx;
     if (!(a->w_bf16 && (Cred % 8 == 0) && aligned16(a->w_bf16))) return 0;
@@ -850,6 +851,10 @@
         int rc = SAVP_OK;
         if (conv_gate_try(a, st, &rc)) return rc;
     }
+    if (a->mode == SAVP_CONV_DGRAD) {
+        int rc = SAVP_OK;
+        if (conv_gate_dgrad_try(a, st, &rc)) return rc;
+    }
     if (a->mode == SAVP_CONV_FPROP || a->mode == SAVP_CONV_DGRAD) {
         const bool dg = a->mode == SAVP_CONV_DGRAD;
         p.out = (float*)(dg ? a->x : a->y);
diff --git a/video_prediction_amd/csrc/opts.h b/video_prediction_amd/csrc/opts.h
--- a/video_prediction_amd/csrc/opts.h
+++ b/video_prediction_amd/csrc/opts.h
@@ -20,6 +20,7 @@
     OPT_GATE_ALT,
     OPT_GATE_CELL,
     OPT_GATE_WWARM,
+    OPT_GATE_DGRAD,
     OPT_SPLITK_REDUCED,
     OPT_COUNT
 };
diff --git a/video_prediction_amd/engine.py b/video_prediction_amd/engine.py
--- a/video_prediction_amd/engine.py
+++ b/video_prediction_amd/engine.py
@@ -249,6 +249,8 @@
         self.need_wt = self.need_wd = True
         self.wfrag = None
         self.wfrag_il = None
+        self.wfrag_d = None
+        self.wfrag_d_gap = None
         self.prof = None
         self.ktimer = None
 
@@ -286,16 +288,30 @@
             K.pack_weights(**entry)
         if self.wfrag is not None and b16:
             K.pack_gate_weights(src, self.wfrag)
-            if self.wfrag_il is not None:
-                K.pack_gate_weights(src, self.wfrag_il, interleave=True)
-
-    def enable_gate_pack(self, cell=False):
+        if self.wfrag_il is not None and b16:
+            K.pack_gate_weights(src, self.wfrag_il, interleave=True)
+        if self.wfrag_d is not None and b16:
+            K.pack_gate_weights_dgrad(src, self.wfrag_d, self.wfrag_d_gap)
+
+    def enable_gate_pack(self, side, cell=False):
         if self.kind == 'conv' and not self.padded and not self.sn_u_name:
             n = K.gate_weights_elems(self.taps, self.cx, self.cy)
-            if n:
+            if n and K.gate_pack_ok('fwd', side, self.cx, self.cy):
                 self.wfrag = torch.empty(n, device=self.W.device, dtype=torch.bfloat16)
-                if cell and self.cy % 32 == 0:
-                    self.wfrag_il = torch.empty(n, device=self.W.device, dtype=torch.bfloat16)
+            if n and cell and K.gate_pack_ok('cell', side, self.cx, self.cy):
+                self.wfrag_il = torch.empty(n, device=self.W.device, dtype=torch.bfloat16)
+
+    def enable_gate_dgrad_pack(self, side, skip=None):
+        if self.kind == 'conv' and not self.padded and not self.sn_u_name:
+            skip = (int(skip[0]), int(skip[1])) if skip is not None and skip[1] else None
+            if K.gate_pack_ok('dgrad', side, self.cx, self.cy, skip):
+                n = K.gate_weights_elems(self.taps, self.cy, self.cx - (skip[1] if skip else 0))
+                self.wfrag_d = torch.empty(n, device=self.W.device, dtype=torch.bfloat16)
+                self.wfrag_d_gap = skip
+
+    def _frag_d(self, dx, skip):
+        skip = (int(skip[0]), int(skip[1])) if skip is not None and skip[1] else None
+        return self.wfrag_d if (self.wfrag_d is not None and dx.shape[-1] == self.cx and skip == self.wfrag_d_gap) else None
 
     def commit_u(self):
         if self.sn_u_name:
@@ -343,7 +359,7 @@
             return K.conv(lib.CONV_FPROP, self.geom, dy, dx, self.wt, beta=beta, act=act, alpha=alpha, aux=aux, w16=self.wt16, dst_gap=skip,
                           norm_bwd=norm_bwd, defer=defer)
         return K.conv(lib.CONV_DGRAD, self.geom, dx, dy, self.wd, beta=beta, act=act, alpha=alpha, aux=aux, w16=self.wd16, dst_gap=skip,
-                      norm_bwd=norm_bwd, defer=defer)
+                      norm_bwd=norm_bwd, defer=defer, w_frag_d=self._frag_d(dx, skip))
 
     def norm_bwd_ok(self, dy, dx, norm_bwd, skip=None):
         if K.PRECISION['value'] != 1:
@@ -351,7 +367,7 @@
         nb = dict(norm_bwd, ws=None)
         if self.kind in TRANSPOSED:
             return K.conv_stats_ok(lib.CONV_FPROP, self.geom, dy, dx, self.wt, w16=self.wt16, dst_gap=skip, norm_bwd=nb)
-        return K.conv_stats_ok(lib.CONV_DGRAD, self.geom, dx, dy, self.wd, w16=self.wd16, dst_gap=skip, norm_bwd=nb)
+        return K.conv_stats_ok(lib.CONV_DGRAD, self.geom, dx, dy, self.wd, w16=self.wd16, dst_gap=skip, norm_bwd=nb, w_frag_d=self._frag_d(dx, skip))
 
     def backward_weights(self, x, dy, feeds_instance_norm=False):
         target = self.dwfp if self.padded else (self.dwf if self.dwf is not None else self.dW)
diff --git a/video_prediction_amd/kernels.py b/video_prediction_amd/kernels.py
--- a/video_prediction_amd/kernels.py
+++ b/video_prediction_amd/kernels.py
@@ -84,7 +84,7 @@
 
 
 def _fill_conv_args(mode, geom, x, y, w, bias, beta, act, alpha, aux, splitk, tile, precision, w16=None, stats=None, dst_gap=None,
-                    norm_bwd=None, w_frag=None, w_frag_il=None):
+                    norm_bwd=None, w_frag=None, w_frag_il=None, w_frag_d=None):
     a = lib.SavpConvArgs()
     a.mode = mode
     N, D, H, W, Cx, a.x_sn, a.x_sd, a.x_sh, a.x_sw = _nd(x)
@@ -125,6 +125,7 @@
     a.stats = stats.data_ptr() if stats is not None else None
     a.w_frag = w_frag.data_ptr() if w_frag is not None else None
     a.w_frag_il = w_frag_il.data_ptr() if w_frag_il is not None else None
+    a.w_frag_d = w_frag_d.data_ptr() if w_frag_d is not None else None
     taps = geom.k[0] * geom.k[1] * geom.k[2]
     if w.numel() != taps * Cx * Cy:
         raise ValueError('weight has %d elements, expected %d' % (w.numel(), taps * Cx * Cy))
@@ -285,11 +286,11 @@
 
 
 def conv(mode, geom, x, y, w, bias=None, beta=0, act=0, alpha=0.0, aux=None, splitk=0, tile=0, precision=None, w16=None, stats=None,
-         dst_gap=None, norm_bwd=None, defer=False, w_frag=None, w_frag_il=None):
+         dst_gap=None, norm_bwd=None, defer=False, w_frag=None, w_frag_il=None, w_frag_d=None):
     lib.require_device(w, bias, aux)
     lib.require_stats(stats, (norm_bwd or {}).get('ws'))
     lib.require_device_any(x, y)
-    a = _fill_conv_args(mode, geom, x, y, w, bias, beta, act, alpha, aux, splitk, tile, precision, w16, stats, dst_gap, norm_bwd, w_frag, w_frag_il)
+    a = _fill_conv_args(mode, geom, x, y, w, bias, beta, act, alpha, aux, splitk, tile, precision, w16, stats, dst_gap, norm_bwd, w_frag, w_frag_il, w_frag_d)
     if AUTOTUNE['enabled'] and tile == 0 and splitk == 0 and not lib.get().savp_conv_special(ctypes.byref(a)):
         key = (mode, a.precision, a.N, a.D, a.H, a.W, a.Cx, a.Do, a.Ho, a.Wo, a.Cy, geom.k, geom.s, geom.p, a.act, a.beta,
                a.x_sw, a.y_sw, bias is not None, w16 is not None, a.src_bf16, a.out_bf16, stats is not None)
@@ -342,8 +343,8 @@
              '/sw%d' % a.y_sw, a.tile, a.splitk, a.act, a.beta, 1 if a.bias else 0))
 
 
-def conv_stats_ok(mode, geom, x, y, w, bias=None, w16=None, dst_gap=None, norm_bwd=None):
-    a = _fill_conv_args(mode, geom, x, y, w, bias, 0, 0, 0.0, None, 0, 0, None, w16, None, dst_gap, norm_bwd)
+def conv_stats_ok(mode, geom, x, y, w, bias=None, w16=None, dst_gap=None, norm_bwd=None, w_frag_d=None):
+    a = _fill_conv_args(mode, geom, x, y, w, bias, 0, 0, 0.0, None, 0, 0, None, w16, None, dst_gap, norm_bwd, w_frag_d=w_frag_d)
     return bool(lib.get().savp_conv_stats_ok(ctypes.byref(a)))
 
 
@@ -1196,6 +1197,24 @@
     lib.check(_L().savp_pack_gate_weights(lib.stream(), _p(src), taps, Cx, Cy, _p(out), int(bool(interleave))), 'savp_pack_gate_weights')
 
 
+def gate_pack_ok(kind, side, Cx, Cy, gap=None):
+    if kind == 'dgrad':
+        g0, g1 = (int(gap[0]), int(gap[1])) if gap is not None and gap[1] else (0, 0)
+        return bool(_L().savp_gate_pack_dgrad_ok(int(side), int(Cx), int(Cy), g0, g1))
+    fn = {'fwd': _L().savp_gate_pack_fwd_ok, 'cell': _L().savp_gate_pack_cell_ok}[kind]
+    return bool(fn(int(side), int(Cx), int(Cy)))
+
+
+def pack_gate_weights_dgrad(src, out, gap=None):
+    lib.require_device(src)
+    Cx, Cy = src.shape[-2], src.shape[-1]
+    taps = src.numel() // (Cx * Cy)
+    g0, g1 = (int(gap[0]), int(gap[1])) if gap is not None and gap[1] else (0, 0)
+    if out.dtype != torch.bfloat16 or out.numel() != gate_weights_elems(taps, Cy, Cx - g1) or not out.numel():
+        raise ValueError('gate weight pack (data gradient): expected %d bf16 elements' % gate_weights_elems(taps, Cy, Cx - g1))
+    lib.check(_L().savp_pack_gate_weights_dgrad(lib.stream(), _p(src), taps, Cx, Cy, g0, g1, _p(out)), 'savp_pack_gate_weights_dgrad')
+
+
 def fold_pool(inp, out, k, adjoint=False):
     C = (out.numel() if adjoint else inp.numel()) // (k * k)
     lib.check(_L().savp_fold_pool(lib.stream(), _p(inp), _p(out), k, C, int(adjoint)), 'savp_fold_pool')
diff --git a/video_prediction_amd/lib.py b/video_prediction_amd/lib.py
--- a/video_prediction_amd/lib.py
+++ b/video_prediction_amd/lib.py
@@ -31,7 +31,7 @@
         ('dst_gap_at', c_i32), ('dst_gap', c_i32),
         ('nb_x', c_vp), ('nb_x_sn', c_i64), ('nb_x_sp', c_i64), ('nb_mean', c_vp), ('nb_rstd', c_vp), ('nb_gamma', c_vp), ('nb_beta', c_vp),
         ('nb_ws', c_vp), ('nb_c0', c_i32), ('nb_nc', c_i32), ('nb_act', c_i32), ('nb_alpha', c_f32),
-        ('w_frag', c_vp), ('w_frag_il', c_vp),
+        ('w_frag', c_vp), ('w_frag_il', c_vp), ('w_frag_d', c_vp),
     ]
 
 
@@ -90,7 +90,7 @@
 
 
 OPTION_NAMES = ('conv_ring', 's2dgrad', 'thin', 'wgp_cfg', 'wgp_split', 'inorm_min_hw', 'colsum_2stage', 'dense_legacy', 'cdna_legacy',
-                'lstm_fused', 'ring_dma', 'lstm_q', 'ring_wwarm', 'wgp_dma', 'ring_early', 'gate_kernel', 'gate_alt', 'gate_cell', 'gate_wwarm', 'splitk_reduced')
+                'lstm_fused', 'ring_dma', 'lstm_q', 'ring_wwarm', 'wgp_dma', 'ring_early', 'gate_kernel', 'gate_alt', 'gate_cell', 'gate_wwarm', 'gate_dgrad', 'splitk_reduced')
 
 
 def set_option(name, value):
@@ -453,6 +453,10 @@
 register('savp_state_pred_fwd', [c_vp, c_i32, c_i32, c_i32, c_i32] + [c_vp] * 7)
 register('savp_state_pred_bwd', [c_vp, c_i32, c_i32, c_i32, c_i32] + [c_vp] * 6)
 register('savp_pack_gate_weights', [c_vp, c_vp, c_i32, c_i32, c_i32, c_vp, c_i32])
+register('savp_pack_gate_weights_dgrad', [c_vp, c_vp, c_i32, c_i32, c_i32, c_i32, c_i32, c_vp])
+register('savp_gate_pack_fwd_ok', [c_i32, c_i32, c_i32])
+register('savp_gate_pack_cell_ok', [c_i32, c_i32, c_i32])
+register('savp_gate_pack_dgrad_ok', [c_i32, c_i32, c_i32, c_i32, c_i32])
 register('savp_debug_poison_lds', [c_vp, ctypes.c_uint32, c_vp])
 register('savp_debug_fill_u32', [c_vp, c_vp, c_i64, ctypes.c_uint32])
 register('savp_debug_probe_lds', [c_vp, ctypes.c_uint32, c_vp])
diff --git a/video_prediction_amd/models/savp_cell.py b/video_prediction_amd/models/savp_cell.py
--- a/video_prediction_amd/models/savp_cell.py
+++ b/video_prediction_amd/models/savp_cell.py
@@ -250,7 +250,7 @@
                 L['dc'] = [torch.empty(N, h_, w_, f, device=dev), torch.empty(N, h_, w_, f, device=dev)] if g else None
                 L['rconv'] = ConvLayer(store, r + 'kernel', (r + 'bias') if self.cell_plain else None, 'conv', (5, 5), (1, 1), (2, 2))
                 if not self.cell_plain and not self.cell_ln:
-                    L['rconv'].enable_gate_pack(cell=bool(L['fused']) and h_ * w_ <= 256)
+                    L['rconv'].enable_gate_pack(h_ if h_ == w_ else 0, cell=bool(L['fused']) and h_ * w_ <= 256)
                 if self.cell_ln:
                     L['gn4'] = ConcatNorm([Norm(store, r + nm + '/', T1, N, f, dev, groups=1) for nm in ('input', 'transform', 'forget', 'output')],
                                           T1, N, dev)
@@ -268,6 +268,8 @@
                                   K.tiled_z_ok(h_, w_, 4 * f, zr, L['rconv'].geom))
                 if L['zless']:
                     L['weff'] = torch.empty(25, 4 * f, K.tiled_z_pad(zr), device=dev)
+                if g and L['fused'] and not self.cell_plain and not self.cell_ln:
+                    L['rconv'].enable_gate_dgrad_pack(h_ if h_ == w_ else 0, skip=(f, zr) if L['zless'] else None)
             else:
                 L['out'] = None
             self.layers.append(L)
```

New measurement: 10530 (median of 6 runs). About the same (+0.5%).
